# facebookresearch/EgoT2

Measured on NVIDIA B200. Metric: translator fwd+bwd clips/sec, higher is better.
Workload: dtype bf16

## Files before the change

### egot2_b200/_lib.py

```python
from __future__ import annotations

import ctypes as C
import os

MAX_SEG = 8
MAX_GROUPS = 4
F32, BF16 = 0, 1
LOSS_NONE, LOSS_CE, LOSS_BCE_SIGMOID, LOSS_CE_GROUPS = 0, 1, 2, 3
LR_CONSTANT, LR_COSINE, LR_STEPS = 0, 1, 2
LR_MAX_MILESTONES = 8

_LIB_PATH = os.environ.get("EGOT2_LIB") or os.path.join(os.path.dirname(os.path.abspath(__file__)), "lib", "libegot2.so")

i32, u64, f32, vp, sz = C.c_int32, C.c_uint64, C.c_float, C.c_void_p, C.c_size_t


class EmbedDesc(C.Structure):
    _fields_ = [("dtype", i32), ("feat_dtype", i32), ("B", i32), ("T", i32), ("H", i32), ("n_seg", i32),
                ("seg_tokens", i32 * MAX_SEG), ("seg_in_dim", i32 * MAX_SEG), ("seg_offset", i32 * MAX_SEG),
                ("seg_has_proj", i32 * MAX_SEG), ("training", i32), ("p_feat", f32), ("p_embed", f32),
                ("ln_eps", f32), ("seed", u64), ("no_ln", i32), ("feat_drop_tokens", i32)]


class EmbedIn(C.Structure):
    _fields_ = [("feat", vp * MAX_SEG), ("proj_w", vp * MAX_SEG), ("proj_b", vp * MAX_SEG), ("ln_g", vp),
                ("ln_b", vp), ("tok_table", vp)]


class EmbedOut(C.Structure):
    _fields_ = [("z", vp), ("stat", vp), ("x", vp)]


class EmbedGrads(C.Structure):
    _fields_ = [("proj_w", vp * MAX_SEG), ("proj_b", vp * MAX_SEG), ("ln_g", vp), ("ln_b", vp), ("tok_table", vp),
                ("dfeat", vp * MAX_SEG), ("seg_embed", vp * MAX_SEG)]


class LayerDesc(C.Structure):
    _fields_ = [("dtype", i32), ("B", i32), ("T", i32), ("H", i32), ("FF", i32), ("heads", i32), ("training", i32),
                ("layer_index", i32), ("p_drop", f32), ("ln_eps", f32), ("seed", u64)]


_LAYER_FIELDS = ["in_proj_w", "out_proj_w", "lin1_w", "lin2_w", "in_proj_b", "out_proj_b", "lin1_b", "lin2_b",
                 "norm1_g", "norm1_b", "norm2_g", "norm2_b"]


class LayerParams(C.Structure):
    _fields_ = [(n, vp) for n in _LAYER_FIELDS]


class LayerGrads(C.Structure):
    _fields_ = [(n, vp) for n in _LAYER_FIELDS]


class LayerSaved(C.Structure):
    _fields_ = [(n, vp) for n in ["qkv", "attn", "lse", "y1", "stat1", "x1", "hid", "y2", "stat2", "hid_mask", "ffn_scratch"]]


class DecoderDesc(C.Structure):
    _fields_ = [("dtype", i32), ("rows", i32), ("S", i32), ("mem_rows", i32), ("M", i32), ("kv_inner", i32),
                ("kv_outer", i32), ("kv_jstride", i32), ("kv_istride", i32), ("H", i32), ("FF", i32), ("heads", i32),
                ("training", i32), ("layer_index", i32), ("p_drop", f32), ("ln_eps", f32), ("seed", u64)]


_DEC_FIELDS = ["sa_in_w", "sa_out_w", "ca_in_w", "ca_out_w", "lin1_w", "lin2_w", "sa_in_b", "sa_out_b", "ca_in_b",
               "ca_out_b", "lin1_b", "lin2_b", "norm1_g", "norm1_b", "norm2_g", "norm2_b", "norm3_g", "norm3_b"]


class DecoderParams(C.Structure):
    _fields_ = [(n, vp) for n in _DEC_FIELDS]


class DecoderGrads(C.Structure):
    _fields_ = [(n, vp) for n in _DEC_FIELDS]


class DecoderSaved(C.Structure):
    _fields_ = [(n, vp) for n in ["qkv", "a1", "y1", "stat1", "x1", "qc", "kvc", "a2", "y2", "stat2", "x2", "hid", "y3",
                                  "stat3"]]


class HeadDesc(C.Structure):
    _fields_ = [("dtype", i32), ("B", i32), ("T", i32), ("H", i32), ("pool", i32), ("row_tokens", i32),
                ("use_ln", i32), ("n_out", i32), ("loss", i32), ("n_groups", i32), ("group_size", i32 * MAX_GROUPS),
                ("sub_rows", i32), ("training", i32), ("p_head", f32), ("ln_eps", f32), ("seed", u64)]


class HeadIn(C.Structure):
    _fields_ = [(n, vp) for n in ["x", "ln_g", "ln_b", "w", "b", "labels", "class_weight"]]


class HeadOut(C.Structure):
    _fields_ = [(n, vp) for n in ["pooled", "stat", "g", "logits", "loss", "argmax", "row_loss"]]


class DpDesc(C.Structure):
    _fields_ = [("world", i32), ("rank", i32), ("numel", C.c_int64), ("slab", vp * 8), ("off_param", C.c_int64),
                ("off_grad", C.c_int64), ("off_shadow", C.c_int64), ("off_flags", C.c_int64), ("exp_avg", vp), ("exp_avg_sq", vp),
                ("lr", f32), ("beta1", f32), ("beta2", f32), ("eps", f32), ("weight_decay", f32), ("step", i32), ("step_dev", vp),
                ("decoupled", i32), ("zero_grads_remote", i32), ("lr_dev", vp), ("guard", vp)]


class GradGuard(C.Structure):
    _fields_ = [("max_norm", f32), ("total_norm", f32), ("coef", f32), ("skip", i32), ("skipped", i32)]


class LrSched(C.Structure):
    _fields_ = [("kind", i32), ("n_milestones", i32), ("warmup_steps", C.c_int64), ("total_steps", C.c_int64),
                ("base_lr", C.c_double), ("warmup_start_lr", C.c_double), ("end_lr", C.c_double),
                ("milestones", C.c_int64 * LR_MAX_MILESTONES), ("factors", C.c_double * (LR_MAX_MILESTONES + 1))]


class HeadGrads(C.Structure):
    _fields_ = [(n, vp) for n in ["ln_g", "ln_b", "w", "b"]]


class VitDesc(C.Structure):
    _fields_ = [("dtype", i32), ("B", i32), ("T", i32), ("D", i32), ("heads", i32), ("dim_head", i32), ("mlp", i32),
                ("layer_index", i32), ("ln_eps", f32)]


_VIT_PARAM_FIELDS = ["qkv_w", "out_w", "ff1_w", "ff2_w", "norm_a_g", "norm_a_b", "norm_f_g", "norm_f_b", "ff1_b", "ff2_b"]


class VitParams(C.Structure):
    _fields_ = [(n, vp) for n in _VIT_PARAM_FIELDS]


class VitGrads(C.Structure):
    _fields_ = [(n, vp) for n in _VIT_PARAM_FIELDS]


class VitSaved(C.Structure):
    _fields_ = [(n, vp) for n in ["h", "stat_a", "qkv", "attn", "lse", "x1", "h2", "stat_f", "u", "act"]]


P = C.POINTER

SIGNATURES = {
    "egot2_version": (C.c_char_p, []),
    "egot2_last_error": (C.c_char_p, []),
    "egot2_sm_count": (C.c_int, []),
    "egot2_launch_count": (C.c_uint64, []),
    "egot2_dropout_epoch_enable": (C.c_int, [C.c_int]),
    "egot2_dropout_epoch_set": (C.c_int, [u64, vp]),
    "egot2_dropout_epoch_advance": (C.c_int, [vp]),
    "egot2_dropout_epoch_host": (C.c_int, [u64]),
    "egot2_pnr_metrics": (C.c_int, [i32, i32, vp, vp, vp, vp, vp, vp, vp, vp, vp, vp, vp, vp]),
    "egot2_row_softmax": (C.c_int, [C.c_int64, i32, vp, vp, vp]),
    "egot2_segment_softmax_mean": (C.c_int, [i32, i32, vp, vp, vp, vp]),
    "egot2_topk_correct": (C.c_int, [i32, i32, vp, vp, i32, vp, vp, vp]),
    "egot2_edit_distance_prefix": (C.c_int, [i32, i32, i32, vp, vp, vp, vp, vp]),
    "egot2_prof_enable": (C.c_int, [C.c_int]),
    "egot2_peer_alloc": (C.c_int, [C.c_size_t, C.POINTER(vp)]),
    "egot2_peer_free": (C.c_int, [vp]),
    "egot2_peer_handle_bytes": (C.c_int, []),
    "egot2_peer_export": (C.c_int, [vp, vp]),
    "egot2_peer_import": (C.c_int, [vp, C.POINTER(vp)]),
    "egot2_peer_unimport": (C.c_int, [vp]),
    "egot2_dp_flag_bytes": (C.c_size_t, []),
    "egot2_dp_reduce_adam": (C.c_int, [vp, vp]),
    "egot2_dp_reduce_adam_range": (C.c_int, [vp, C.c_int64, C.c_int64, i32, vp]),
    "egot2_side_defer": (C.c_int, [C.c_int]),
    "egot2_side_join_all": (C.c_int, [vp]),
    "egot2_timeline_set": (C.c_int, [vp]),
    "egot2_prof_report": (C.c_int, [C.c_char_p, sz]),
    "egot2_embed_workspace_bytes": (sz, [P(EmbedDesc), C.c_int]),
    "egot2_embed_fwd": (C.c_int, [P(EmbedDesc), P(EmbedIn), P(EmbedOut), vp, sz, vp]),
    "egot2_embed_bwd": (C.c_int, [P(EmbedDesc), P(EmbedIn), P(EmbedOut), vp, P(EmbedGrads), vp, sz, vp]),
    "egot2_hhi_tok_table_fwd": (C.c_int, [vp, vp, i32, i32, P(i32), P(i32), i32, vp, vp]),
    "egot2_hhi_tok_table_bwd": (C.c_int, [vp, i32, P(i32), P(i32), i32, vp, vp]),
    "egot2_ffn_scratch_bytes": (sz, [i32]),
    "egot2_encoder_layer_workspace_bytes": (sz, [P(LayerDesc), C.c_int]),
    "egot2_encoder_layer_fwd": (C.c_int, [P(LayerDesc), P(LayerParams), vp, vp, P(LayerSaved), vp, sz, vp]),
    "egot2_encoder_layer_bwd": (C.c_int, [P(LayerDesc), P(LayerParams), vp, P(LayerSaved), vp, vp, P(LayerGrads),
                                          vp, sz, vp]),
    "egot2_decoder_layer_workspace_bytes": (sz, [P(DecoderDesc)]),
    "egot2_decoder_layer_fwd": (C.c_int, [P(DecoderDesc), P(DecoderParams), vp, vp, vp, P(DecoderSaved), vp]),
    "egot2_decoder_layer_bwd": (C.c_int, [P(DecoderDesc), P(DecoderParams), vp, vp, P(DecoderSaved), vp, vp, vp,
                                          P(DecoderGrads), vp, sz, vp]),
    "egot2_vit_layer_workspace_bytes": (sz, [P(VitDesc)]),
    "egot2_vit_layer_fwd": (C.c_int, [P(VitDesc), P(VitParams), vp, vp, P(VitSaved), vp]),
    "egot2_vit_layer_bwd": (C.c_int, [P(VitDesc), P(VitParams), vp, P(VitSaved), vp, vp, P(VitGrads), vp, sz, vp]),
    "egot2_prompt_embed_fwd": (C.c_int, [i32, i32, i32, i32, vp, vp, vp, f32, i32, u64, vp, vp]),
    "egot2_prompt_embed_bwd": (C.c_int, [i32, i32, i32, i32, vp, vp, f32, i32, u64, vp, vp]),
    "egot2_head_rows": (C.c_int, [P(HeadDesc)]),
    "egot2_head_workspace_bytes": (sz, [P(HeadDesc)]),
    "egot2_head_loss_fwd": (C.c_int, [P(HeadDesc), P(HeadIn), P(HeadOut), vp]),
    "egot2_head_loss_bwd": (C.c_int, [P(HeadDesc), P(HeadIn), P(HeadOut), vp, f32, vp, P(HeadGrads), vp, sz, vp]),
    "egot2_slowfast_pool_fwd": (C.c_int, [vp, i32, i32, i32, i32, i32, i32, vp, i32, vp]),
    "egot2_cast_f32_to_bf16": (C.c_int, [vp, vp, sz, vp]),
    "egot2_sum_into_f32": (C.c_int, [vp, vp, vp, sz, vp]),
    "egot2_cast_bf16_to_f32": (C.c_int, [vp, vp, sz, vp]),
    "egot2_adam_step": (C.c_int, [vp, vp, vp, vp, sz, f32, f32, f32, f32, f32, i32, f32, vp]),
    "egot2_adam_step_fused": (C.c_int, [vp, vp, vp, vp, sz, f32, f32, f32, f32, f32, i32, f32, vp, i32, vp]),
    "egot2_adamw_step_fused": (C.c_int, [vp, vp, vp, vp, sz, f32, f32, f32, f32, f32, i32, f32, vp, i32, vp]),
    "egot2_adam_step_fused_dev": (C.c_int, [vp, vp, vp, vp, sz, f32, f32, f32, f32, f32, vp, f32, vp, i32, vp]),
    "egot2_adam_step_fused_sched": (C.c_int, [vp, vp, vp, vp, sz, vp, f32, f32, f32, f32, vp, f32, vp, i32, i32, vp]),
    "egot2_opt_advance": (C.c_int, [vp, vp, vp, vp]),
    "egot2_grad_norm_workspace_bytes": (sz, []),
    "egot2_grad_norm": (C.c_int, [vp, sz, f32, vp, vp, vp, sz, vp]),
    "egot2_adam_step_fused_guard": (C.c_int, [vp, vp, vp, vp, sz, f32, vp, f32, f32, f32, f32, vp, f32, vp, i32, i32, vp, vp]),
    "egot2_gemm": (C.c_int, [i32, i32, i32, i32, vp, i32, vp, i32, vp, i32, vp, i32, i32, vp]),
    "egot2_gemm_last_impl": (C.c_char_p, []),
    "egot2_layernorm_fwd": (C.c_int, [i32, i32, i32, vp, vp, vp, f32, vp, vp, vp]),
    "egot2_attention_fwd": (C.c_int, [i32, i32, i32, i32, i32, vp, vp, vp, f32, i32, u64, vp]),
    "egot2_attention_bwd": (C.c_int, [i32, i32, i32, i32, i32, vp, vp, vp, vp, vp, f32, i32, u64, vp, sz, vp]),
    "egot2_attention_bwd_workspace_bytes": (sz, [i32, i32, i32, i32, i32]),
    "egot2_pool_fwd": (C.c_int, [i32, i32, i32, i32, i32, i32, vp, vp, vp]),
    "egot2_pool_bwd": (C.c_int, [i32, i32, i32, i32, i32, i32, vp, vp, vp]),
}

_lib = None


class Egot2Error(RuntimeError):
    pass


def lib_path() -> str:
    return _LIB_PATH


def load():
    global _lib
    if _lib is not None:
        return _lib
    if not os.path.exists(_LIB_PATH):
        raise Egot2Error(f"{_LIB_PATH} not found: build it with `python -m egot2_b200.build` "
                         "(the CUDA library is mandatory; there is no PyTorch/CPU fallback)")
    lib = C.CDLL(_LIB_PATH)
    for name, (res, args) in SIGNATURES.items():
        fn = getattr(lib, name)
        fn.restype = res
        fn.argtypes = args
    _lib = lib
    return lib


def check(rc: int, what: str = ""):
    if rc != 0:
        msg = load().egot2_last_error().decode(errors="replace")
        raise Egot2Error(f"{what or 'egot2 call'} failed (rc={rc}): {msg}")


def call(name: str, *args):
    check(getattr(load(), name)(*args), name)


def prof_enable(on: bool = True):
    check(load().egot2_prof_enable(1 if on else 0), "egot2_prof_enable")


def prof_report():
    buf = C.create_string_buffer(1 << 20)
    check(load().egot2_prof_report(buf, len(buf)), "egot2_prof_report")
    rows = []
    for line in buf.value.decode().splitlines():
        tag, n, us = line.split("\t")
        rows.append((tag, int(n), float(us)))
    return sorted(rows, key=lambda r: -r[2])
```

### egot2_b200/csrc/api.cu

```cuda
#include <stdarg.h>
#include <stdlib.h>
#include <string.h>

#define EGOT2_FILE_ID 11
#include "ops.h"

namespace egot2 {

static thread_local char g_err[512] = "";
unsigned long long g_launch_count = 0;

void set_error(const char* fmt, ...) {
  va_list ap;
  va_start(ap, fmt);
  vsnprintf(g_err, sizeof(g_err), fmt, ap);
  va_end(ap);
}

#ifdef EGOT2_TIMELINE
static void (*g_tl_setters[32])(unsigned long long*);
static int g_tl_n = 0;
void tl_register(void (*setter)(unsigned long long*)) { if (g_tl_n < 32) g_tl_setters[g_tl_n++] = setter; }
#endif

unsigned long long g_host_epoch = 0;
static void (*g_epoch_setters[32])(const unsigned long long*);
static int g_epoch_n = 0;
void epoch_register(void (*setter)(const unsigned long long*)) { if (g_epoch_n < 32) g_epoch_setters[g_epoch_n++] = setter; }
namespace {
__global__ void epoch_advance_kernel(unsigned long long* slot, unsigned long long add) {
  EGOT2_PDL_ENTER();
  if (threadIdx.x == 0 && blockIdx.x == 0) *slot += add;
}
constexpr int kMaxDev = 64;
unsigned long long* g_epoch_slots[kMaxDev] = {};
int cur_dev() { int d = 0; return (cudaGetDevice(&d) == cudaSuccess && d >= 0 && d < kMaxDev) ? d : 0; }
#define g_epoch_slot (g_epoch_slots[cur_dev()])
}

bool pdl_enabled() {
  static const bool on = !(getenv("EGOT2_PDL") && atoi(getenv("EGOT2_PDL")) == 0);
  return on;
}

int sm_count() {
  static int cached[64] = {0};
  int dev = 0;
  if (cudaGetDevice(&dev) != cudaSuccess || dev < 0 || dev >= 64) return 148;
  if (cached[dev] == 0) {
    int n = 0;
    if (cudaDeviceGetAttribute(&n, cudaDevAttrMultiProcessorCount, dev) != cudaSuccess || n <= 0) n = 148;
    cached[dev] = n;
  }
  return cached[dev];
}

int suggest_split_k(int M, int N, int K) {
  const int tile = (M <= 64 || N <= 64) ? 64 : 128;
  const long long tiles = (long long)((M + tile - 1) / tile) * ((N + tile - 1) / tile);
  long long want = (2LL * sm_count() + tiles - 1) / tiles;
  long long max_by_k = K / 128;
  if (want > max_by_k) want = max_by_k;
  if (want < 1) want = 1;
  if (want > 64) want = 64;
  return (int)want;
}

namespace {
struct ProfRec { char tag[96]; cudaEvent_t e0, e1; };
constexpr int kProfMax = 16384;
ProfRec* g_prof = nullptr;
int g_prof_n = 0;
bool g_prof_on = false;
}
bool prof_enabled() { return g_prof_on; }
ProfScope::ProfScope(cudaStream_t stream, const char* fmt, ...) : st(stream), slot(-1) {
  static const bool trace = getenv("EGOT2_TRACE_LAUNCH") != nullptr;
  if (trace) {
    char tag[96];
    va_list ap;
    va_start(ap, fmt);
    vsnprintf(tag, sizeof(tag), fmt, ap);
    va_end(ap);
    fprintf(stderr, "[egot2] %s\n", tag);
    fflush(stderr);
  }
  if (!g_prof_on || g_prof_n >= kProfMax) return;
  cudaStreamCaptureStatus cs = cudaStreamCaptureStatusNone;
  if (cudaStreamIsCapturing(stream, &cs) != cudaSuccess || cs != cudaStreamCaptureStatusNone) return;
  ProfRec& r = g_prof[g_prof_n];
  if (!r.e0) { if (cudaEventCreate(&r.e0) != cudaSuccess || cudaEventCreate(&r.e1) != cudaSuccess) return; }
  va_list ap;
  va_start(ap, fmt);
  vsnprintf(r.tag, sizeof(r.tag), fmt, ap);
  va_end(ap);
  slot = g_prof_n++;
  cudaEventRecord(r.e0, st);
}
ProfScope::~ProfScope() {
  if (slot >= 0) cudaEventRecord(g_prof[slot].e1, st);
}

static thread_local const char* g_gemm_impl = "none";
const char* gemm_last_impl() { return g_gemm_impl; }

static int gemm_impl_mode() {
  static int mode = -1;
  if (mode < 0) {
    const char* e = getenv("EGOT2_GEMM");
    mode = (e && strcmp(e, "simt") == 0) ? 1 : 0;
  }
  return mode;
}

int gemm(const GemmArgs& a, cudaStream_t st) {
  if (a.in_dtype == EGOT2_BF16 && gemm_impl_mode() == 0) {
    const int rc = gemm_sm100(a, st);
    if (rc >= 0) { if (rc == 0) g_gemm_impl = "tcgen05"; return rc; }
  }
  g_gemm_impl = "simt";
  EGOT2_CHECK(!a.trans_c, "gemm: transposed accumulation exists in the tcgen05 kernel only");
  EGOT2_CHECK(a.ln_g == nullptr, "gemm: a fused LayerNorm was requested but the tcgen05 kernel did not take the problem");
  if (a.split_stride > 0) {
    GemmArgs b = a;
    b.split_k = 1; b.split_stride = 0;
    if (a.splits_out) *a.splits_out = 1;
    return gemm_simt(b, st);
  }
  return gemm_simt(a, st);
}

static bool env_is(const char* name, const char* value) {
  const char* e = getenv(name);
  return e && strcmp(e, value) == 0;
}

static bool force_simt_attention() {
  static int mode = -1;
  if (mode < 0) { const char* e = getenv("EGOT2_ATTN"); mode = (e && strcmp(e, "simt") == 0) ? 1 : 0; }
  return mode == 1;
}

int attention_fwd(int dtype, int B, int T, int H, int heads, const void* qkv, void* out, float* lse, float p_drop,
                  uint64_t drop_key, cudaStream_t st) {
  if (heads > 0 && H % heads == 0 && H / heads > 128)
    return attention_wide_fwd(dtype, B, T, H, heads, qkv, out, lse, p_drop, drop_key, st);
  if (attention_mma_supported(dtype, T, H, heads) && !force_simt_attention())
    return attention_mma_fwd(B, T, H, heads, qkv, out, lse, p_drop, drop_key, st);
  if (attention_long_supported(dtype, T, H, heads) && !force_simt_attention())
    return attention_long_fwd(B, T, H, heads, qkv, out, lse, p_drop, drop_key, st);
  return attention_simt_fwd(dtype, B, T, H, heads, qkv, out, lse, p_drop, drop_key, st);
}
int attention_bwd(int dtype, int B, int T, int H, int heads, const void* qkv, const void* out, const float* lse,
                  const void* dout, void* dqkv, float p_drop, uint64_t drop_key, void* ws, size_t ws_bytes,
                  cudaStream_t st) {
  if (heads > 0 && H % heads == 0 && H / heads > 128)
    return attention_wide_bwd(dtype, B, T, H, heads, qkv, out, lse, dout, dqkv, p_drop, drop_key, st);
  if (attention_mma_supported(dtype, T, H, heads) && !force_simt_attention())
    return attention_mma_bwd(B, T, H, heads, qkv, out, lse, dout, dqkv, p_drop, drop_key, st);
  if (attention_long_supported(dtype, T, H, heads) && !force_simt_attention())
    return attention_long_bwd(B, T, H, heads, qkv, out, lse, dout, dqkv, p_drop, drop_key, st);
  return attention_simt_bwd(dtype, B, T, H, heads, qkv, out, lse, dout, dqkv, p_drop, drop_key, ws, ws_bytes, st);
}

namespace {

struct Carver {
  char* base; size_t size, off = 0;
  Carver(void* p, size_t n) : base((char*)p), size(n) {}
  void* take(size_t bytes) {
    void* r = base ? base + off : nullptr;
    off += align_up(bytes);
    return r;
  }
  bool ok() const { return off <= size && (base != nullptr || off == 0); }
};

struct Side {
  cudaStream_t s = nullptr;
  cudaEvent_t fork[8] = {};
  cudaEvent_t join = nullptr;
  cudaEvent_t pend[2] = {};
  const void* pend_ws[2] = {nullptr, nullptr};
  int pend_next = 0;
  bool dirty = false;
};
int g_side_defer[kMaxDev] = {};
constexpr int kCallers = 4;
struct SideSets {
  Side sides[kCallers][3];
  cudaStream_t owner[kCallers] = {};
  unsigned long long used[kCallers] = {};
  unsigned long long tick = 0;
  int state = 0;
};
SideSets g_side_sets[kMaxDev];
Side* get_side(int idx, cudaStream_t caller) {
  SideSets& ss = g_side_sets[cur_dev()];
  if (ss.state == 0) {
    ss.state = 1;
    if (env_is("EGOT2_STREAMS", "0")) ss.state = -1;
    for (int c = 0; c < kCallers && ss.state == 1; ++c)
      for (int i = 0; i < 3 && ss.state == 1; ++i) {
        Side& sd = ss.sides[c][i];
        if (cudaStreamCreateWithFlags(&sd.s, cudaStreamNonBlocking) != cudaSuccess) ss.state = -1;
        for (int k = 0; k < 8 && ss.state == 1; ++k)
          if (cudaEventCreateWithFlags(&sd.fork[k], cudaEventDisableTiming) != cudaSuccess) ss.state = -1;
        if (ss.state == 1 && cudaEventCreateWithFlags(&sd.join, cudaEventDisableTiming) != cudaSuccess) ss.state = -1;
        for (int k = 0; k < 2 && ss.state == 1; ++k)
          if (cudaEventCreateWithFlags(&sd.pend[k], cudaEventDisableTiming) != cudaSuccess) ss.state = -1;
      }
  }
  if (ss.state != 1) return nullptr;
  int slot = -1, lru = 0;
  for (int c = 0; c < kCallers; ++c) {
    if (ss.used[c] && ss.owner[c] == caller) { slot = c; break; }
    if (ss.used[c] < ss.used[lru]) lru = c;
  }
  if (slot < 0) { slot = lru; ss.owner[slot] = caller; }
  ss.used[slot] = ++ss.tick;
  return &ss.sides[slot][idx];
}
}
int launch_priority(cudaStream_t st) {
  static int state = 0, lo = 0, hi = 0;
  if (state == 0) {
    state = 1;
    if (env_is("EGOT2_PRIO", "0") || cudaDeviceGetStreamPriorityRange(&lo, &hi) != cudaSuccess || lo == hi) state = -1;
  }
  if (state != 1) return INT_MIN;
  {
    const SideSets& ss = g_side_sets[cur_dev()];
    if (ss.state == 1)
      for (int c = 0; c < kCallers; ++c)
        for (int i = 0; i < 3; ++i)
          if (ss.sides[c][i].s == st) return lo;
  }
  return hi;
}
namespace {
cudaStream_t side_fork(cudaStream_t main, Side* sd, int k) {
  if (!sd || prof_enabled()) return main;
  if (cudaEventRecord(sd->fork[k], main) != cudaSuccess || cudaStreamWaitEvent(sd->s, sd->fork[k], 0) != cudaSuccess) return main;
  return sd->s;
}
int side_join(cudaStream_t main, Side* sd) {
  if (!sd || prof_enabled()) return 0;
  EGOT2_CUDA(cudaEventRecord(sd->join, sd->s));
  EGOT2_CUDA(cudaStreamWaitEvent(main, sd->join, 0));
  sd->dirty = false;
  sd->pend_ws[0] = sd->pend_ws[1] = nullptr;
  return 0;
}
bool side_deferred() { return g_side_defer[cur_dev()] != 0 && !prof_enabled(); }
int side_mark_pending(Side* sd, const void* ws) {
  if (!sd) return 0;
  int slot = sd->pend_ws[0] == ws ? 0 : sd->pend_ws[1] == ws ? 1 : (sd->pend_next++ & 1);
  EGOT2_CUDA(cudaEventRecord(sd->pend[slot], sd->s));
  sd->pend_ws[slot] = ws;
  sd->dirty = true;
  return 0;
}
int side_wait_pending(cudaStream_t main, Side* sd, const void* ws) {
  if (!sd) return 0;
  for (int k = 0; k < 2; ++k)
    if (sd->pend_ws[k] == ws) {
      EGOT2_CUDA(cudaStreamWaitEvent(main, sd->pend[k], 0));
      sd->pend_ws[k] = nullptr;
    }
  return 0;
}

int wgrad(int dtype, int rows, int n_out, int k_in, const void* dY, int ld_dy, int dy_rpg, int dy_gs, const void* X,
          int ld_x, int x_rpg, int x_gs, float* dW, cudaStream_t st, int share = 1) {
  static const bool swap_on = !env_is("EGOT2_WGRAD_SWAP", "0");
  if (swap_on && dtype == EGOT2_BF16 && gemm_impl_mode() == 0 && k_in <= 128 && n_out >= 512 && !dy_rpg && !x_rpg && share == 1) {
    GemmArgs t;
    t.M = k_in; t.N = n_out; t.K = rows;
    t.A = X; t.lda = ld_x; t.trans_a = 1;
    t.B = dY; t.ldb = ld_dy; t.trans_b = 0;
    t.C = dW; t.ldc = k_in; t.trans_c = 1; t.in_dtype = dtype; t.out_dtype = EGOT2_F32; t.accumulate = 1;
    t.split_k = suggest_split_k(t.M, t.N, t.K);
    const int rc = t.split_k >= 2 ? gemm_sm100(t, st) : -3;
    if (rc >= 0) return rc;
  }
  GemmArgs g;
  g.M = n_out; g.N = k_in; g.K = rows;
  g.A = dY; g.lda = ld_dy; g.trans_a = 1; g.a_rpg = dy_rpg; g.a_gstride = dy_gs;
  g.B = X; g.ldb = ld_x; g.trans_b = 0; g.b_rpg = x_rpg; g.b_gstride = x_gs;
  g.C = dW; g.ldc = k_in; g.in_dtype = dtype; g.out_dtype = EGOT2_F32; g.accumulate = 1;
  g.split_k = suggest_split_k(g.M, g.N, g.K);
  if (share > 1) g.split_k = g.split_k / share > 0 ? g.split_k / share : 1;
  return gemm(g, st);
}

}
}

using namespace egot2;

extern "C" const char* egot2_version(void) { return "egot2-b200 0.1 (sm_100a)"; }
extern "C" const char* egot2_last_error(void) { return g_err; }
extern "C" int egot2_sm_count(void) { return sm_count(); }
extern "C" uint64_t egot2_launch_count(void) { return g_launch_count; }

extern "C" int egot2_timeline_set(void* dev_buf) {
#ifdef EGOT2_TIMELINE
  for (int i = 0; i < g_tl_n; ++i) g_tl_setters[i]((unsigned long long*)dev_buf);
  return 0;
#else
  (void)dev_buf;
  EGOT2_CHECK(false, "this build has no timeline support (compile with -DEGOT2_TIMELINE)");
#endif
}

extern "C" int egot2_dropout_epoch_enable(int on) {
  if (on && !g_epoch_slot) {
    EGOT2_CUDA(cudaMalloc(&g_epoch_slot, sizeof(unsigned long long)));
    EGOT2_CUDA(cudaMemset(g_epoch_slot, 0, sizeof(unsigned long long)));
  }
  const unsigned long long* p = on ? g_epoch_slot : nullptr;
  for (int i = 0; i < g_epoch_n; ++i) g_epoch_setters[i](p);
  EGOT2_CUDA(cudaGetLastError());
  return 0;
}
extern "C" int egot2_dropout_epoch_set(uint64_t value, void* stream) {
  EGOT2_CHECK(g_epoch_slot != nullptr, "dropout epoch: call egot2_dropout_epoch_enable(1) first");
  EGOT2_CUDA(cudaMemsetAsync(g_epoch_slot, 0, sizeof(unsigned long long), (cudaStream_t)stream));
  if (value) {
    launch(epoch_advance_kernel, dim3(1), dim3(32), 0, (cudaStream_t)stream, g_epoch_slot, (unsigned long long)value);
    EGOT2_LAUNCH_CHECK();
  }
  return 0;
}
extern "C" int egot2_dropout_epoch_advance(void* stream) {
  EGOT2_CHECK(g_epoch_slot != nullptr, "dropout epoch: call egot2_dropout_epoch_enable(1) first");
  launch(epoch_advance_kernel, dim3(1), dim3(32), 0, (cudaStream_t)stream, g_epoch_slot, 1ull);
  EGOT2_LAUNCH_CHECK();
  return 0;
}
extern "C" int egot2_dropout_epoch_host(uint64_t value) { g_host_epoch = value; return 0; }

extern "C" int egot2_pnr_metrics(int32_t B, int32_t n, const float* logits, const int64_t* label_idx,
                                 const float* label_onehot, const int64_t* sc_label, const double* fps,
                                 const int64_t* start_frame, const int64_t* end_frame, const int64_t* pnr_frame,
                                 double* err_sec, int64_t* out_counts, double* out_dist_sum, void* stream) {
  return pnr_metrics(B, n, logits, label_idx, label_onehot, sc_label, fps, start_frame, end_frame, pnr_frame, err_sec,
                     (long long*)out_counts, out_dist_sum, (cudaStream_t)stream);
}

extern "C" int egot2_prof_enable(int on) {
  if (on && !g_prof) {
    g_prof = (ProfRec*)calloc(kProfMax, sizeof(ProfRec));
    EGOT2_CHECK(g_prof != nullptr, "prof: out of host memory");
  }
  g_prof_on = on != 0;
  if (on) g_prof_n = 0;
  return 0;
}
extern "C" int egot2_prof_report(char* buf, size_t buf_bytes) {
  EGOT2_CHECK(buf && buf_bytes > 0, "prof_report: no buffer");
  struct Agg { const char* tag; int n; double us; };
  Agg* agg = (Agg*)calloc(g_prof_n > 0 ? g_prof_n : 1, sizeof(Agg));
  int na = 0;
  for (int i = 0; i < g_prof_n; ++i) {
    float ms = 0.f;
    EGOT2_CUDA(cudaEventSynchronize(g_prof[i].e1));
    EGOT2_CUDA(cudaEventElapsedTime(&ms, g_prof[i].e0, g_prof[i].e1));
    int j = 0;
    for (; j < na; ++j) if (strcmp(agg[j].tag, g_prof[i].tag) == 0) break;
    if (j == na) { agg[na].tag = g_prof[i].tag; agg[na].n = 0; agg[na].us = 0; ++na; }
    agg[j].n += 1; agg[j].us += ms * 1e3;
  }
  size_t off = 0;
  buf[0] = 0;
  for (int j = 0; j < na; ++j) {
    int w = snprintf(buf + off, buf_bytes - off, "%s\t%d\t%.3f\n", agg[j].tag, agg[j].n, agg[j].us);
    if (w < 0 || (size_t)w >= buf_bytes - off) break;
    off += w;
  }
  free(agg);
  return 0;
}

namespace {
void seg_stream_plan(const egot2_embed_desc* d, int* idx) {
  long long load[3] = {0, 0, 0};
  bool done[EGOT2_MAX_SEG] = {};
  for (int it = 0; it < d->n_seg; ++it) {
    int best = -1;
    long long bc = -1;
    for (int k = 0; k < d->n_seg; ++k) {
      if (done[k]) continue;
      const long long c = d->seg_has_proj[k] ? (long long)d->seg_in_dim[k] * d->seg_tokens[k] : 1;
      if (c > bc) { bc = c; best = k; }
    }
    int sidx = 0;
    for (int j = 1; j < 3; ++j) if (load[j] < load[sidx]) sidx = j;
    idx[best] = sidx;
    load[sidx] += bc;
    done[best] = true;
  }
}

bool embed_splitk(const egot2_embed_desc* d) {
  if (env_is("EGOT2_EMBED_SPLITK", "0")) return false;
  if (d->no_ln || !embed_finish_supported(d->dtype, d->H)) return false;
  if (env_is("EGOT2_EMBED_SPLITK", "1")) return true;
  for (int k = 0; k < d->n_seg; ++k) {
    if (!d->seg_has_proj[k] || d->seg_tokens[k] == 0) continue;
    const long long tiles = (((long long)d->B * d->seg_tokens[k] + 127) / 128) * ((d->H + 127) / 128);
    if (d->seg_in_dim[k] >= 2048 && tiles * 2 <= sm_count()) return true;
  }
  return false;
}
int embed_seg_splits(const egot2_embed_desc* d, int k) {
  if (!d->seg_has_proj[k] || d->seg_tokens[k] == 0) return 1;
  const long long tiles = (((long long)d->B * d->seg_tokens[k] + 127) / 128) * ((d->H + 127) / 128);
  long long s = sm_count() / tiles;
  if (s > d->seg_in_dim[k] / 512) s = d->seg_in_dim[k] / 512;
  if (s > 16) s = 16;
  return s < 1 ? 1 : (int)s;
}
size_t embed_slab_floats(const egot2_embed_desc* d) {
  size_t n = 0;
  for (int k = 0; k < d->n_seg; ++k)
    if (d->seg_has_proj[k]) n += (size_t)embed_seg_splits(d, k) * d->B * d->seg_tokens[k] * d->H;
  return n;
}
}

extern "C" size_t egot2_embed_workspace_bytes(const egot2_embed_desc* d, int backward) {
  size_t n = 256;
  if (!backward && embed_splitk(d)) n += align_up(embed_slab_floats(d) * 4);
  if (!backward && d->feat_dtype != d->dtype) {
    size_t mx = 0;
    for (int k = 0; k < d->n_seg; ++k) {
      const size_t e = (size_t)d->B * d->seg_tokens[k] * d->seg_in_dim[k];
      if (e > mx) mx = e;
    }
    n += align_up(mx * dtype_size(d->dtype));
  }
  if (backward && d->feat_dtype != d->dtype) {
    size_t mx = 0;
    for (int k = 0; k < d->n_seg; ++k) {
      const size_t e = (size_t)d->B * d->seg_tokens[k] * d->seg_in_dim[k];
      if (e > mx) mx = e;
    }
    n += align_up(mx * dtype_size(d->dtype));
  }
  if (backward) n += align_up((size_t)d->B * d->T * d->H * dtype_size(d->dtype));
  return n;
}

static int embed_check(const egot2_embed_desc* d) {
  EGOT2_CHECK(d->n_seg >= 1 && d->n_seg <= EGOT2_MAX_SEG, "embed: n_seg=%d out of range", d->n_seg);
  EGOT2_CHECK(d->dtype == EGOT2_F32 || d->dtype == EGOT2_BF16, "embed: bad dtype %d", d->dtype);
  EGOT2_CHECK(d->feat_dtype == d->dtype || (d->feat_dtype == EGOT2_F32 && d->dtype == EGOT2_BF16),
              "embed: features must be in the compute dtype, or fp32 with bf16 compute");
  int tot = 0;
  for (int k = 0; k < d->n_seg; ++k) {
    EGOT2_CHECK(d->seg_offset[k] == tot, "embed: segment %d offset %d != running total %d", k, d->seg_offset[k], tot);
    EGOT2_CHECK(d->seg_has_proj[k] || d->seg_in_dim[k] == d->H, "embed: pass-through segment %d must be H wide", k);
    tot += d->seg_tokens[k];
  }
  EGOT2_CHECK(tot == d->T, "embed: segments cover %d tokens, T=%d", tot, d->T);
  EGOT2_CHECK(!d->no_ln || !d->training || (d->p_feat == 0.f && d->p_embed == 0.f),
              "embed: the LayerNorm-free variant has no dropout sites (p_feat=%f p_embed=%f)", d->p_feat, d->p_embed);
  return 0;
}

extern "C" int egot2_embed_fwd(const egot2_embed_desc* d, const egot2_embed_in* in, const egot2_embed_out* out,
                               void* workspace, size_t ws_bytes, void* stream) {
  cudaStream_t st = (cudaStream_t)stream;
  EGOT2_TRY(embed_check(d));
  if (d->B == 0 || d->T == 0) return 0;
  const size_t es = dtype_size(d->dtype);
  Carver ws(workspace, ws_bytes);
  void* cast_buf = nullptr;
  const bool splitk = embed_splitk(d);
  float* zf = nullptr;
  EmbedSrc src;
  src.n = d->n_seg;
  if (splitk) {
    zf = (float*)ws.take(embed_slab_floats(d) * 4);
    EGOT2_CHECK(ws.ok(), "embed_fwd: workspace too small (%zu < %zu)", ws_bytes, ws.off);
  }
  if (d->feat_dtype != d->dtype) {
    size_t mx = 0;
    for (int k = 0; k < d->n_seg; ++k) {
      const size_t e = (size_t)d->B * d->seg_tokens[k] * d->seg_in_dim[k];
      if (e > mx) mx = e;
    }
    cast_buf = ws.take(mx * dtype_size(d->dtype));
    EGOT2_CHECK(ws.ok(), "embed_fwd: workspace too small (%zu < %zu)", ws_bytes, ws.off);
  }
  const bool par = d->feat_dtype == d->dtype;
  Side* sides[2] = {par ? get_side(0, st) : nullptr, par ? get_side(1, st) : nullptr};
  bool used[2] = {false, false};
  cudaStream_t side_st[2] = {st, st};
  int seg_idx[EGOT2_MAX_SEG] = {};
  seg_stream_plan(d, seg_idx);
  for (int i = 0; i < 2 && i + 1 < d->n_seg; ++i)
    if (sides[i]) { side_st[i] = side_fork(st, sides[i], 0); used[i] = side_st[i] != st; }
  bool ln_fused = !splitk && !d->no_ln && d->dtype == EGOT2_BF16 && d->feat_dtype == EGOT2_BF16 && d->H == 128 &&
                  !(d->training && d->p_feat > 0.f) && gemm_impl_mode() == 0 && env_is("EGOT2_GEMM_LN", "1");
  for (int k = 0; k < d->n_seg && ln_fused; ++k)
    if (d->seg_tokens[k] > 0 && (!d->seg_has_proj[k] || d->seg_in_dim[k] % 8 != 0)) ln_fused = false;
  for (int k = 0; k < d->n_seg; ++k) {
    const int Dk = d->seg_tokens[k], Kk = d->seg_in_dim[k];
    if (Dk == 0) continue;
    cudaStream_t sk = seg_idx[k] > 0 ? side_st[seg_idx[k] - 1] : st;
    char* zk = (char*)out->z + (size_t)d->seg_offset[k] * d->H * es;
    const void* feat = in->feat[k];
    if (splitk && !d->seg_has_proj[k]) {
      src.direct[k] = feat; src.direct_f32[k] = d->feat_dtype == EGOT2_F32 && d->dtype != EGOT2_F32;
      continue;
    }
    if (d->feat_dtype != d->dtype) {
      EGOT2_TRY(cast_f32_to(d->dtype, (const float*)feat, cast_buf, (size_t)d->B * Dk * Kk, sk));
      feat = cast_buf;
    }
    if (d->seg_has_proj[k]) {
      GemmArgs g;
      g.M = d->B * Dk; g.N = d->H; g.K = Kk;
      g.A = feat; g.lda = Kk;
      g.B = in->proj_w[k]; g.ldb = Kk; g.trans_b = 1;
      g.C = zk; g.ldc = d->H; g.c_rpg = Dk; g.c_gstride = d->T;
      g.bias = in->proj_b[k];
      g.in_dtype = d->dtype; g.out_dtype = d->dtype;
      if (splitk) {
        g.C = zf; g.ldc = d->H; g.c_rpg = 0; g.c_gstride = 0; g.out_dtype = EGOT2_F32;
        g.split_k = embed_seg_splits(d, k); g.split_stride = (long long)d->B * Dk * d->H;
        int used = 1;
        g.splits_out = &used;
        EGOT2_TRY(gemm(g, sk));
        src.slab[k] = zf; src.splits[k] = used;
        zf += (size_t)embed_seg_splits(d, k) * d->B * Dk * d->H;
      } else {
        if (ln_fused) {
          g.ln_g = in->ln_g; g.ln_b = in->ln_b; g.ln_eps = d->ln_eps;
          g.ln_out = (char*)out->x + (size_t)d->seg_offset[k] * d->H * es; g.ln_stat = out->stat;
          g.ln_table = in->tok_table; g.ln_table_rows = d->T; g.ln_row0 = d->seg_offset[k];
          if (d->training && d->p_embed > 0.f) { g.ln_p_drop = d->p_embed; g.ln_drop_key = site_key(d->seed, SITE_EMBED, 0); }
          if (!gemm_sm100_ln_ok(g)) {
            ln_fused = false;
            g.ln_g = nullptr; g.ln_b = nullptr; g.ln_out = nullptr; g.ln_stat = nullptr; g.ln_table = nullptr; g.ln_p_drop = 0.f;
          }
        }
        EGOT2_TRY(gemm(g, sk));
      }
    } else {
      EGOT2_CUDA(cudaMemcpy2DAsync(zk, (size_t)d->T * d->H * es, feat, (size_t)Dk * d->H * es, (size_t)Dk * d->H * es,
                                   d->B, cudaMemcpyDeviceToDevice, sk));
    }
  }
  for (int i = 0; i < 2; ++i) if (used[i]) EGOT2_TRY(side_join(st, sides[i]));
  const size_t n = (size_t)d->B * d->T * d->H;
  if (splitk) {
    for (int k = 0; k < d->n_seg; ++k) { src.tok_begin[k] = d->seg_offset[k]; src.tokens[k] = d->seg_tokens[k]; }
    return embed_finish(d->B, d->T, d->H, src, (d->feat_drop_tokens > 0 && d->feat_drop_tokens < d->T) ? d->feat_drop_tokens : 0,
                        d->training ? d->p_feat : 0.f, site_key(d->seed, SITE_FEAT, 0), in->ln_g, in->ln_b, d->ln_eps, in->tok_table,
                        d->training ? d->p_embed : 0.f, site_key(d->seed, SITE_EMBED, 0), out->z, out->stat, out->x, st);
  }
  if (d->training && d->p_feat > 0.f) {
    if (d->feat_drop_tokens > 0 && d->feat_drop_tokens < d->T)
      EGOT2_TRY(dropout_prefix_inplace(d->dtype, out->z, n, (size_t)d->T * d->H, (size_t)d->feat_drop_tokens * d->H, d->p_feat,
                                       site_key(d->seed, SITE_FEAT, 0), st));
    else
      EGOT2_TRY(dropout_inplace(d->dtype, out->z, n, d->p_feat, site_key(d->seed, SITE_FEAT, 0), st));
  }
  if (d->no_ln) return add_table(d->dtype, n, (size_t)d->T * d->H, out->z, in->tok_table, out->x, st);
  if (ln_fused) return 0;
  LayerNormArgs l;
  l.rows = d->B * d->T; l.H = d->H; l.dtype = d->dtype; l.x = out->z; l.g = in->ln_g; l.b = in->ln_b; l.eps = d->ln_eps;
  l.y = out->x; l.stat = out->stat; l.table = in->tok_table; l.table_rows = d->T;
  if (d->training && d->p_embed > 0.f) { l.p_drop = d->p_embed; l.drop_key = site_key(d->seed, SITE_EMBED, 0); }
  return layernorm_fwd(l, st);
}

extern "C" int egot2_embed_bwd(const egot2_embed_desc* d, const egot2_embed_in* in, const egot2_embed_out* saved,
                               const void* dx_c, const egot2_embed_grads* g, void* workspace, size_t ws_bytes,
                               void* stream) {
  cudaStream_t st = (cudaStream_t)stream;
  EGOT2_TRY(embed_check(d));
  if (d->B == 0 || d->T == 0) return 0;
  void* dx = const_cast<void*>(dx_c);
  const size_t es = dtype_size(d->dtype);
  const size_t n = (size_t)d->B * d->T * d->H;
  Carver ws(workspace, ws_bytes);
  void* cast_buf = nullptr;
  if (d->feat_dtype != d->dtype) {
    size_t mx = 0;
    for (int k = 0; k < d->n_seg; ++k) {
      const size_t e = (size_t)d->B * d->seg_tokens[k] * d->seg_in_dim[k];
      if (e > mx) mx = e;
    }
    cast_buf = ws.take(mx * es);
  }
  void* dz = ws.take(n * es);
  EGOT2_CHECK(ws.ok(), "embed_bwd: workspace too small (%zu < %zu)", ws_bytes, ws.off);
  const float pe = (d->training && d->p_embed > 0.f) ? d->p_embed : 0.f;
  const uint64_t ke = site_key(d->seed, SITE_EMBED, 0);
  SegOut so;
  so.n = d->n_seg;
  bool want_table = g->tok_table != nullptr;
  for (int k = 0; k < d->n_seg; ++k) { so.tokens[k] = d->seg_tokens[k]; so.out[k] = g->seg_embed[k]; want_table |= g->seg_embed[k] != nullptr; }
  Side* tside = want_table ? get_side(2, st) : nullptr;
  if (want_table) EGOT2_TRY(table_grad(d->dtype, d->B, d->T, d->H, dx, g->tok_table, so, pe, ke, side_fork(st, tside, 0)));
  if (d->no_ln) {
    dz = dx;
  } else {
    LayerNormBwdArgs l;
    l.rows = d->B * d->T; l.H = d->H; l.dtype = d->dtype; l.x = saved->z; l.stat = saved->stat; l.g = in->ln_g;
    l.dy = dx; l.dx = dz; l.dg = g->ln_g; l.db = g->ln_b; l.dy_p_drop = pe; l.dy_drop_key = ke;
    EGOT2_TRY(layernorm_bwd(l, st));
    if (d->training && d->p_feat > 0.f) {
      if (d->feat_drop_tokens > 0 && d->feat_drop_tokens < d->T)
        EGOT2_TRY(dropout_prefix_inplace(d->dtype, dz, n, (size_t)d->T * d->H, (size_t)d->feat_drop_tokens * d->H, d->p_feat,
                                         site_key(d->seed, SITE_FEAT, 0), st));
      else
        EGOT2_TRY(dropout_inplace(d->dtype, dz, n, d->p_feat, site_key(d->seed, SITE_FEAT, 0), st));
    }
  }
  const bool par = d->feat_dtype == d->dtype;
  Side* sides[2] = {par ? get_side(0, st) : nullptr, par ? get_side(1, st) : nullptr};
  bool used[2] = {false, false};
  cudaStream_t side_st[2] = {st, st};
  int seg_idx[EGOT2_MAX_SEG] = {};
  seg_stream_plan(d, seg_idx);
  for (int i = 0; i < 2 && i + 1 < d->n_seg; ++i)
    if (sides[i]) { side_st[i] = side_fork(st, sides[i], 0); used[i] = side_st[i] != st; }
  int n_proj = 0, n_big = 0;
  long long sum_big = 0;
  for (int k = 0; k < d->n_seg; ++k) {
    const bool on = d->seg_has_proj[k] && d->seg_tokens[k] > 0;
    n_proj += on ? 1 : 0;
    n_big += (on && d->seg_in_dim[k] >= 2048) ? 1 : 0;
    if (on && d->seg_in_dim[k] >= 2048) sum_big += (long long)d->seg_in_dim[k] * d->seg_tokens[k];
  }
  const int share_all = n_big > 0 ? n_big : n_proj;
  auto big_share = [&](int Kk, int Dk) {
    const long long w = (long long)Kk * Dk;
    const long long sh = w > 0 ? (sum_big + w / 2) / w : 1;
    return (int)(sh < 1 ? 1 : sh);
  };
  bool bias_on_main = false;
  SegOut sb_main;
  {
    SegOut sb;
    sb.n = d->n_seg;
    bool any = false;
    for (int k = 0; k < d->n_seg; ++k) {
      sb.tokens[k] = d->seg_tokens[k];
      sb.out[k] = (d->seg_has_proj[k] && d->seg_tokens[k] > 0) ? g->proj_b[k] : nullptr;
      any |= sb.out[k] != nullptr;
    }
    Side* bside = get_side(2, st);
    if (any && tside) {
      bias_on_main = true;
      sb_main = sb;
    } else if (any) {
      EGOT2_TRY(table_grad(d->dtype, d->B, d->T, d->H, dz, nullptr, sb, 0.f, 0, side_fork(st, bside, 1)));
      if (bside && !tside) tside = bside;
    }
  }
  for (int k = 0; k < d->n_seg; ++k) {
    const int Dk = d->seg_tokens[k], Kk = d->seg_in_dim[k];
    if (Dk == 0) continue;
    cudaStream_t sk = seg_idx[k] > 0 ? side_st[seg_idx[k] - 1] : st;
    const char* dzk = (const char*)dz + (size_t)d->seg_offset[k] * d->H * es;
    if (d->seg_has_proj[k]) {
      const void* feat = in->feat[k];
      if (d->feat_dtype != d->dtype) {
        EGOT2_TRY(cast_f32_to(d->dtype, (const float*)feat, cast_buf, (size_t)d->B * Dk * Kk, sk));
        feat = cast_buf;
      }
      if (g->proj_w[k])
        EGOT2_TRY(wgrad(d->dtype, d->B * Dk, d->H, Kk, dzk, d->H, Dk, d->T, feat, Kk, 0, 0, g->proj_w[k], sk,
                        !par ? 1 : ((n_big > 0 && Kk < 2048) ? 8 : (n_big > 0 ? big_share(Kk, Dk) : share_all))));
      if (g->dfeat[k]) {
        GemmArgs m;
        m.M = d->B * Dk; m.N = Kk; m.K = d->H;
        m.A = dzk; m.lda = d->H; m.a_rpg = Dk; m.a_gstride = d->T;
        m.B = in->proj_w[k]; m.ldb = Kk; m.trans_b = 0;
        m.C = g->dfeat[k]; m.ldc = Kk; m.in_dtype = d->dtype; m.out_dtype = EGOT2_F32;
        EGOT2_TRY(gemm(m, sk));
      }
    } else if (g->dfeat[k]) {
      if (d->dtype == EGOT2_F32) {
        EGOT2_CUDA(cudaMemcpy2DAsync(g->dfeat[k], (size_t)Dk * d->H * 4, dzk, (size_t)d->T * d->H * 4,
                                     (size_t)Dk * d->H * 4, d->B, cudaMemcpyDeviceToDevice, sk));
      } else {
        for (int b = 0; b < d->B; ++b)
          EGOT2_TRY(cast_to_f32(d->dtype, dzk + (size_t)b * d->T * d->H * es, g->dfeat[k] + (size_t)b * Dk * d->H,
                                (size_t)Dk * d->H, sk));
      }
    }
  }
  if (bias_on_main) EGOT2_TRY(table_grad(d->dtype, d->B, d->T, d->H, dz, nullptr, sb_main, 0.f, 0, st));
  for (int i = 0; i < 2; ++i) if (used[i]) EGOT2_TRY(side_join(st, sides[i]));
  if (tside) EGOT2_TRY(side_join(st, tside));
  return 0;
}

namespace {
struct LayerWs {
  void *d1, *d2, *d3, *d4, *d5, *dhid, *dqkv, *attn_ws;
  size_t attn_ws_bytes;
};
size_t layer_ws_layout(const egot2_layer_desc* d, int backward, void* base, size_t bytes, LayerWs* out) {
  Carver ws(base, bytes);
  if (backward) {
    const size_t es = dtype_size(d->dtype);
    const size_t M = (size_t)d->B * d->T;
    LayerWs w;
    w.d1 = ws.take(M * d->H * es);
    w.d2 = ws.take(M * d->H * es);
    w.d3 = ws.take(M * d->H * es);
    w.d4 = ws.take(M * d->H * es);
    w.d5 = ws.take(M * d->H * es);
    w.dhid = ws.take(M * d->FF * es);
    w.dqkv = ws.take(M * 3 * d->H * es);
    w.attn_ws_bytes = attention_bwd_workspace(d->dtype, d->B, d->T, d->H, d->heads);
    w.attn_ws = ws.take(w.attn_ws_bytes);
    if (out) *out = w;
  }
  return ws.off + 256;
}
int layer_check(const egot2_layer_desc* d) {
  EGOT2_CHECK(d->dtype == EGOT2_F32 || d->dtype == EGOT2_BF16, "layer: bad dtype %d", d->dtype);
  EGOT2_CHECK(d->heads > 0 && d->H % d->heads == 0, "layer: H=%d not divisible by heads=%d", d->H, d->heads);
  EGOT2_CHECK(d->p_drop >= 0.f && d->p_drop < 1.f, "layer: dropout p=%f out of [0,1)", d->p_drop);
  return 0;
}
}

extern "C" size_t egot2_ffn_scratch_bytes(int32_t M) { return M > 0 ? ffn_scratch_bytes(M) : 0; }

extern "C" size_t egot2_encoder_layer_workspace_bytes(const egot2_layer_desc* d, int backward) {
  return layer_ws_layout(d, backward, nullptr, 0, nullptr);
}

extern "C" int egot2_encoder_layer_fwd(const egot2_layer_desc* d, const egot2_layer_params* p, const void* x_in,
                                       void* x_out, const egot2_layer_saved* s, void* workspace, size_t ws_bytes,
                                       void* stream) {
  (void)workspace; (void)ws_bytes;
  cudaStream_t st = (cudaStream_t)stream;
  EGOT2_TRY(layer_check(d));
  const int M = d->B * d->T, H = d->H, FF = d->FF;
  if (M == 0) return 0;
  const float pd = d->training ? d->p_drop : 0.f;
  const uint32_t L = (uint32_t)d->layer_index;
  bool ln1_fused = false;
  {
    GemmArgs g; g.M = M; g.N = 3 * H; g.K = H; g.A = x_in; g.lda = H; g.B = p->in_proj_w; g.ldb = H; g.trans_b = 1;
    g.C = s->qkv; g.ldc = 3 * H; g.bias = p->in_proj_b; g.in_dtype = d->dtype; g.out_dtype = d->dtype;
    EGOT2_TRY(gemm(g, st));
  }
  EGOT2_TRY(attention_fwd(d->dtype, d->B, d->T, H, d->heads, s->qkv, s->attn, s->lse, pd, site_key(d->seed, SITE_ATTN, L), st));
  {
    GemmArgs g; g.M = M; g.N = H; g.K = H; g.A = s->attn; g.lda = H; g.B = p->out_proj_w; g.ldb = H; g.trans_b = 1;
    g.C = s->y1; g.ldc = H; g.bias = p->out_proj_b; g.residual = x_in; g.ldr = H;
    g.p_drop = pd; g.drop_key = site_key(d->seed, SITE_DROP1, L); g.in_dtype = d->dtype; g.out_dtype = d->dtype;
    g.ln_g = p->norm1_g; g.ln_b = p->norm1_b; g.ln_eps = d->ln_eps; g.ln_out = s->x1; g.ln_stat = s->stat1;
    ln1_fused = d->dtype == EGOT2_BF16 && gemm_sm100_ln_ok(g) && !env_is("EGOT2_GEMM", "simt");
    if (!ln1_fused) { g.ln_g = nullptr; g.ln_b = nullptr; g.ln_out = nullptr; g.ln_stat = nullptr; }
    EGOT2_TRY(gemm(g, st));
  }
  if (!ln1_fused) {
    LayerNormArgs l; l.rows = M; l.H = H; l.dtype = d->dtype; l.x = s->y1; l.g = p->norm1_g; l.b = p->norm1_b;
    l.eps = d->ln_eps; l.y = s->x1; l.stat = s->stat1;
    EGOT2_TRY(layernorm_fwd(l, st));
  }
  if (ffn_fused_supported(d->dtype, H, FF) && !env_is("EGOT2_FFN", "unfused"))
    return ffn_fused_fwd(M, FF, s->x1, p->lin1_w, p->lin1_b, p->lin2_w, p->lin2_b, p->norm2_g, p->norm2_b, d->ln_eps,
                         s->hid, s->hid_mask, s->y2, s->stat2, x_out, pd, site_key(d->seed, SITE_FFN, L),
                         site_key(d->seed, SITE_DROP2, L), s->ffn_scratch, st);
  {
    GemmArgs g; g.M = M; g.N = FF; g.K = H; g.A = s->x1; g.lda = H; g.B = p->lin1_w; g.ldb = H; g.trans_b = 1;
    g.C = s->hid; g.ldc = FF; g.bias = p->lin1_b; g.relu = 1;
    g.p_drop = pd; g.drop_key = site_key(d->seed, SITE_FFN, L); g.drop_bit_mode = 1; g.in_dtype = d->dtype; g.out_dtype = d->dtype;
    EGOT2_TRY(gemm(g, st));
  }
  {
    GemmArgs g; g.M = M; g.N = H; g.K = FF; g.A = s->hid; g.lda = FF; g.B = p->lin2_w; g.ldb = FF; g.trans_b = 1;
    g.C = s->y2; g.ldc = H; g.bias = p->lin2_b; g.residual = s->x1; g.ldr = H;
    g.p_drop = pd; g.drop_key = site_key(d->seed, SITE_DROP2, L); g.in_dtype = d->dtype; g.out_dtype = d->dtype;
    EGOT2_TRY(gemm(g, st));
  }
  {
    LayerNormArgs l; l.rows = M; l.H = H; l.dtype = d->dtype; l.x = s->y2; l.g = p->norm2_g; l.b = p->norm2_b;
    l.eps = d->ln_eps; l.y = x_out; l.stat = s->stat2;
    EGOT2_TRY(layernorm_fwd(l, st));
  }
  return 0;
}

extern "C" int egot2_encoder_layer_bwd(const egot2_layer_desc* d, const egot2_layer_params* p, const void* x_in,
                                       const egot2_layer_saved* s, void* dx_out, void* dx_in,
                                       const egot2_layer_grads* g, void* workspace, size_t ws_bytes, void* stream) {
  cudaStream_t st = (cudaStream_t)stream;
  EGOT2_TRY(layer_check(d));
  const int M = d->B * d->T, H = d->H, FF = d->FF;
  if (M == 0) return 0;
  LayerWs w;
  const size_t need = layer_ws_layout(d, 1, workspace, ws_bytes, &w);
  EGOT2_CHECK(workspace && ws_bytes + 256 >= need, "encoder_layer_bwd: workspace too small (%zu < %zu)", ws_bytes, need);
  const size_t es = dtype_size(d->dtype);
  const float pd = d->training ? d->p_drop : 0.f;
  const float inv_keep = pd > 0.f ? 1.f / (1.f - pd) : 1.f;
  const uint32_t L = (uint32_t)d->layer_index;
  const int dt = d->dtype;

  Side* sd0 = get_side(0, st);
  Side* sd1 = get_side(1, st);
  Side* sd2 = get_side(2, st);
  const bool defer = side_deferred();
  if (defer) {
    EGOT2_TRY(side_wait_pending(st, sd0, workspace));
    EGOT2_TRY(side_wait_pending(st, sd1, workspace));
    EGOT2_TRY(side_wait_pending(st, sd2, workspace));
  }

  const void* d2 = w.d1;
  {
    LayerNormBwdArgs l; l.rows = M; l.H = H; l.dtype = dt; l.x = s->y2; l.stat = s->stat2; l.g = p->norm2_g;
    l.dy = dx_out; l.dx = w.d1; l.dg = g->norm2_g; l.db = g->norm2_b;
    if (pd > 0.f) { l.dx2 = w.d2; l.dx2_p_drop = pd; l.dx2_drop_key = site_key(d->seed, SITE_DROP2, L); d2 = w.d2; }
    l.dcol = g->lin2_b;
    EGOT2_TRY(layernorm_bwd(l, st));
  }
  static const bool late_wgrad = env_is("EGOT2_LATE_WGRAD", "1");
  auto fork_dw2 = [&]() -> int {
    cudaStream_t ss = side_fork(st, sd0, 0);
    return wgrad(dt, M, H, FF, d2, H, 0, 0, s->hid, FF, 0, 0, g->lin2_w, ss);
  };
  if (!late_wgrad) EGOT2_TRY(fork_dw2());
  const bool fused_dx = s->hid_mask && ffn_fused_supported(dt, H, FF) && !env_is("EGOT2_FFN", "unfused");
  if (fused_dx) {
    EGOT2_TRY(ffn_fused_bwd_dx(M, FF, d2, pd > 0.f ? w.d1 : nullptr, s->hid_mask, p->lin1_w, p->lin2_w, pd, w.dhid, w.d3, s->ffn_scratch,
                               g->lin1_b, st));
  } else {
    GemmArgs m; m.M = M; m.N = FF; m.K = H; m.A = d2; m.lda = H; m.B = p->lin2_w; m.ldb = FF; m.trans_b = 0;
    m.C = w.dhid; m.ldc = FF; m.mask = s->hid; m.ldm = FF; m.mask_scale = inv_keep; m.in_dtype = dt; m.out_dtype = dt;
    EGOT2_TRY(gemm(m, st));
    GemmArgs n; n.M = M; n.N = H; n.K = FF; n.A = w.dhid; n.lda = FF; n.B = p->lin1_w; n.ldb = H; n.trans_b = 0;
    n.C = w.d3; n.ldc = H; n.residual = w.d1; n.ldr = H; n.in_dtype = dt; n.out_dtype = dt;
    EGOT2_TRY(gemm(n, st));
  }
  auto fork_dw1 = [&]() -> int {
    cudaStream_t ss = side_fork(st, sd1, 1);
    EGOT2_TRY(wgrad(dt, M, FF, H, w.dhid, FF, 0, 0, s->x1, H, 0, 0, g->lin1_w, ss));
    if (!fused_dx) {
      cudaStream_t s2 = side_fork(st, sd2, 1);
      EGOT2_TRY(colsum_accum(dt, M, FF, w.dhid, FF, 0, 0, g->lin1_b, s2));
    }
    return 0;
  };
  if (!late_wgrad) EGOT2_TRY(fork_dw1());
  const void* dyo = w.d4;
  {
    LayerNormBwdArgs l; l.rows = M; l.H = H; l.dtype = dt; l.x = s->y1; l.stat = s->stat1; l.g = p->norm1_g;
    l.dy = w.d3; l.dx = w.d4; l.dg = g->norm1_g; l.db = g->norm1_b;
    if (pd > 0.f) { l.dx2 = w.d5; l.dx2_p_drop = pd; l.dx2_drop_key = site_key(d->seed, SITE_DROP1, L); dyo = w.d5; }
    l.dcol = g->out_proj_b;
    EGOT2_TRY(layernorm_bwd(l, st));
  }
  if (late_wgrad) { EGOT2_TRY(fork_dw2()); EGOT2_TRY(fork_dw1()); }
  {
    cudaStream_t ss = side_fork(st, sd2, 2);
    EGOT2_TRY(wgrad(dt, M, H, H, dyo, H, 0, 0, s->attn, H, 0, 0, g->out_proj_w, ss));
  }
  {
    GemmArgs m; m.M = M; m.N = H; m.K = H; m.A = dyo; m.lda = H; m.B = p->out_proj_w; m.ldb = H; m.trans_b = 0;
    m.C = w.d3; m.ldc = H; m.in_dtype = dt; m.out_dtype = dt;
    EGOT2_TRY(gemm(m, st));
  }
  EGOT2_TRY(attention_bwd(dt, d->B, d->T, H, d->heads, s->qkv, s->attn, s->lse, w.d3, w.dqkv, pd,
                          site_key(d->seed, SITE_ATTN, L), w.attn_ws, w.attn_ws_bytes, st));
  {
    cudaStream_t ss = side_fork(st, sd0, 3);
    EGOT2_TRY(wgrad(dt, M, 3 * H, H, w.dqkv, 3 * H, 0, 0, x_in, H, 0, 0, g->in_proj_w, ss));
    cudaStream_t s2 = side_fork(st, sd2, 3);
    EGOT2_TRY(colsum_accum(dt, M, 3 * H, w.dqkv, 3 * H, 0, 0, g->in_proj_b, s2));
  }
  {
    GemmArgs m; m.M = M; m.N = H; m.K = 3 * H; m.A = w.dqkv; m.lda = 3 * H; m.B = p->in_proj_w; m.ldb = H; m.trans_b = 0;
    m.C = dx_in; m.ldc = H; m.residual = w.d4; m.ldr = H; m.in_dtype = dt; m.out_dtype = dt;
    EGOT2_TRY(gemm(m, st));
  }
  if (defer) {
    EGOT2_TRY(side_mark_pending(sd0, workspace));
    EGOT2_TRY(side_mark_pending(sd1, workspace));
    return side_mark_pending(sd2, workspace);
  }
  EGOT2_TRY(side_join(st, sd0));
  EGOT2_TRY(side_join(st, sd1));
  return side_join(st, sd2);
}

extern "C" int egot2_side_defer(int on) { g_side_defer[cur_dev()] = on ? 1 : 0; return 0; }

extern "C" int egot2_side_join_all(void* stream) {
  SideSets& ss = g_side_sets[cur_dev()];
  if (ss.state == 1)
    for (int c = 0; c < kCallers; ++c)
      for (int i = 0; i < 3; ++i)
        if (ss.sides[c][i].dirty) EGOT2_TRY(side_join((cudaStream_t)stream, &ss.sides[c][i]));
  return 0;
}

extern "C" int egot2_head_rows(const egot2_head_desc* d) { return d->pool ? d->B : d->B * d->row_tokens; }

extern "C" size_t egot2_head_workspace_bytes(const egot2_head_desc* d) {
  const size_t rows = (size_t)egot2_head_rows(d), es = dtype_size(d->dtype);
  const size_t ldl = ((size_t)d->n_out + 7) / 8 * 8;
  return align_up(rows * ldl * es) + align_up(rows * d->H * es) + align_up(rows * d->H * 4) + 256;
}

extern "C" int egot2_head_loss_fwd(const egot2_head_desc* d, const egot2_head_in* in, const egot2_head_out* out,
                                   void* stream) {
  cudaStream_t st = (cudaStream_t)stream;
  const int rows = egot2_head_rows(d);
  if (rows == 0) return 0;
  EGOT2_CHECK(d->pool || (d->row_tokens > 0 && d->row_tokens <= d->T), "head: row_tokens=%d out of range", d->row_tokens);
  if (head_fused_supported(*d)) {
    if (d->loss != EGOT2_LOSS_NONE)
      EGOT2_CHECK(in->labels && out->row_loss && out->loss, "head_loss_fwd: labels/row_loss/loss buffers required");
    EGOT2_TRY(head_fused_fwd(*d, *in, *out, st));
    return loss_reduce(*d, rows, out->row_loss, out->loss, st);
  }
  EGOT2_TRY(pool_fwd(d->dtype, d->B, d->T, d->H, d->pool, d->row_tokens, in->x, out->pooled, st));
  const float ph = d->training ? d->p_head : 0.f;
  if (d->use_ln) {
    LayerNormArgs l; l.rows = rows; l.H = d->H; l.dtype = d->dtype; l.x = out->pooled; l.x_is_f32 = 1; l.g = in->ln_g;
    l.b = in->ln_b; l.eps = d->ln_eps; l.y = out->g; l.stat = out->stat;
    l.p_drop = ph; l.drop_key = site_key(d->seed, SITE_HEAD, 0);
    EGOT2_TRY(layernorm_fwd(l, st));
  } else {
    EGOT2_TRY(cast_f32_to(d->dtype, out->pooled, out->g, (size_t)rows * d->H, st));
    EGOT2_TRY(dropout_inplace(d->dtype, out->g, (size_t)rows * d->H, ph, site_key(d->seed, SITE_HEAD, 0), st));
  }
  {
    GemmArgs g; g.M = rows; g.N = d->n_out; g.K = d->H; g.A = out->g; g.lda = d->H; g.B = in->w; g.ldb = d->H; g.trans_b = 1;
    g.C = out->logits; g.ldc = d->n_out; g.bias = in->b; g.in_dtype = d->dtype; g.out_dtype = EGOT2_F32;
    EGOT2_TRY(gemm(g, st));
  }
  return loss_fwd(*d, rows, out->logits, in->labels, in->class_weight, out->row_loss, out->loss, out->argmax, st);
}

extern "C" int egot2_head_loss_bwd(const egot2_head_desc* d, const egot2_head_in* in, const egot2_head_out* saved,
                                   float* dlogits, float dloss_scale, void* dx, const egot2_head_grads* g,
                                   void* workspace, size_t ws_bytes, void* stream) {
  cudaStream_t st = (cudaStream_t)stream;
  const int rows = egot2_head_rows(d);
  if (rows == 0) return 0;
  const size_t es = dtype_size(d->dtype);
  if (head_fused_supported(*d))
    return head_fused_bwd(*d, *in, *saved, dlogits, dloss_scale, dx, *g, st);
  EGOT2_CHECK(workspace && ws_bytes >= egot2_head_workspace_bytes(d) - 256, "head_loss_bwd: workspace too small");
  Carver ws(workspace, ws_bytes);
  const int ldl = d->dtype == EGOT2_F32 ? d->n_out : (d->n_out + 7) / 8 * 8;
  void* dl_lp = ws.take((size_t)rows * ldl * es);
  void* dg = ws.take((size_t)rows * d->H * es);
  float* dpooled = (float*)ws.take((size_t)rows * d->H * 4);
  if (d->loss != EGOT2_LOSS_NONE)
    EGOT2_TRY(loss_bwd(*d, rows, saved->logits, in->labels, in->class_weight, saved->loss, dloss_scale, dlogits, st));
  const void* dl = dlogits;
  if (d->dtype != EGOT2_F32) {
    EGOT2_TRY(cast_rows_f32_to_bf16(dlogits, rows, d->n_out, dl_lp, ldl, st));
    dl = dl_lp;
  }
  if (g->w) EGOT2_TRY(wgrad(d->dtype, rows, d->n_out, d->H, dl, ldl, 0, 0, saved->g, d->H, 0, 0, g->w, st));
  if (g->b) EGOT2_TRY(colsum_accum(EGOT2_F32, rows, d->n_out, dlogits, d->n_out, 0, 0, g->b, st));
  const float ph = d->training ? d->p_head : 0.f;
  if (d->dtype == EGOT2_BF16 && !d->use_ln && d->n_out >= 2048 && !env_is("EGOT2_HEAD_SPLITK", "0")) {
    EGOT2_CUDA(cudaMemsetAsync(dpooled, 0, (size_t)rows * d->H * 4, st));
    GemmArgs m; m.M = rows; m.N = d->H; m.K = d->n_out; m.A = dl; m.lda = ldl; m.B = in->w; m.ldb = d->H; m.trans_b = 0;
    m.C = dpooled; m.ldc = d->H; m.in_dtype = d->dtype; m.out_dtype = EGOT2_F32; m.accumulate = 1;
    m.split_k = suggest_split_k(m.M, m.N, m.K);
    EGOT2_TRY(gemm(m, st));
    EGOT2_TRY(dropout_inplace(EGOT2_F32, dpooled, (size_t)rows * d->H, ph, site_key(d->seed, SITE_HEAD, 0), st));
    return pool_bwd(d->dtype, d->B, d->T, d->H, d->pool, d->row_tokens, dpooled, dx, st);
  }
  {
    GemmArgs m; m.M = rows; m.N = d->H; m.K = d->n_out; m.A = dl; m.lda = ldl; m.B = in->w; m.ldb = d->H; m.trans_b = 0;
    m.C = dg; m.ldc = d->H; m.in_dtype = d->dtype; m.out_dtype = d->dtype;
    EGOT2_TRY(gemm(m, st));
  }
  EGOT2_TRY(dropout_inplace(d->dtype, dg, (size_t)rows * d->H, ph, site_key(d->seed, SITE_HEAD, 0), st));
  if (d->use_ln) {
    LayerNormBwdArgs l; l.rows = rows; l.H = d->H; l.dtype = d->dtype; l.x = saved->pooled; l.x_is_f32 = 1;
    l.stat = saved->stat; l.g = in->ln_g; l.dy = dg; l.dy_is_f32 = (d->dtype == EGOT2_F32); l.dx = dpooled; l.dx_is_f32 = 1;
    l.dg = g->ln_g; l.db = g->ln_b;
    EGOT2_TRY(layernorm_bwd(l, st));
  } else {
    EGOT2_TRY(cast_to_f32(d->dtype, dg, dpooled, (size_t)rows * d->H, st));
  }
  return pool_bwd(d->dtype, d->B, d->T, d->H, d->pool, d->row_tokens, dpooled, dx, st);
}

extern "C" int egot2_gemm(int32_t dtype, int32_t M, int32_t N, int32_t K, const void* A, int32_t trans_a, const void* B,
                          int32_t trans_b, const float* bias, int32_t relu, void* C, int32_t c_is_f32,
                          int32_t accumulate, void* stream) {
  GemmArgs g;
  g.M = M; g.N = N; g.K = K;
  g.A = A; g.trans_a = trans_a; g.lda = trans_a ? M : K;
  g.B = B; g.trans_b = trans_b; g.ldb = trans_b ? K : N;
  g.C = C; g.ldc = N; g.bias = bias; g.relu = relu;
  g.in_dtype = dtype; g.out_dtype = c_is_f32 ? EGOT2_F32 : dtype; g.accumulate = accumulate;
  if (accumulate && !relu) g.split_k = suggest_split_k(M, N, K);
  return gemm(g, (cudaStream_t)stream);
}

extern "C" int egot2_sum_into_f32(float* dst, float* a, float* b, size_t n, void* stream) {
  return sum_into_clear(dst, a, b, n, (cudaStream_t)stream);
}

extern "C" const char* egot2_gemm_last_impl(void) { return gemm_last_impl(); }

extern "C" int egot2_attention_fwd(int32_t dtype, int32_t B, int32_t T, int32_t H, int32_t heads, const void* qkv,
                                   void* out, float* lse, float p_drop, int32_t training, uint64_t seed, void* stream) {
  return attention_fwd(dtype, B, T, H, heads, qkv, out, lse, training ? p_drop : 0.f, site_key(seed, SITE_ATTN, 0),
                       (cudaStream_t)stream);
}
extern "C" int egot2_attention_bwd(int32_t dtype, int32_t B, int32_t T, int32_t H, int32_t heads, const void* qkv,
                                   const void* out, const float* lse, const void* dout, void* dqkv, float p_drop,
                                   int32_t training, uint64_t seed, void* workspace, size_t ws_bytes, void* stream) {
  return attention_bwd(dtype, B, T, H, heads, qkv, out, lse, dout, dqkv, training ? p_drop : 0.f,
                       site_key(seed, SITE_ATTN, 0), workspace, ws_bytes, (cudaStream_t)stream);
}
extern "C" size_t egot2_attention_bwd_workspace_bytes(int32_t dtype, int32_t B, int32_t T, int32_t H, int32_t heads) {
  return attention_bwd_workspace(dtype, B, T, H, heads);
}
extern "C" int egot2_pool_fwd(int32_t dtype, int32_t B, int32_t T, int32_t H, int32_t pool, int32_t row_tokens,
                              const void* x, float* pooled, void* stream) {
  return pool_fwd(dtype, B, T, H, pool, row_tokens, x, pooled, (cudaStream_t)stream);
}
extern "C" int egot2_pool_bwd(int32_t dtype, int32_t B, int32_t T, int32_t H, int32_t pool, int32_t row_tokens,
                              const float* dpooled, void* dx, void* stream) {
  return pool_bwd(dtype, B, T, H, pool, row_tokens, dpooled, dx, (cudaStream_t)stream);
}
```

### egot2_b200/csrc/gemm_sm100.cu

```cuda
#include <stdio.h>
#include <stdlib.h>

#define EGOT2_FILE_ID 4
#include "ops.h"
#include "sm100.cuh"

namespace egot2 {

using namespace sm100;

namespace {

constexpr int BM = 128;
constexpr int BK = 64;
#ifndef EGOT2_GEMM_EPG
#define EGOT2_GEMM_EPG 1
#endif
constexpr int EPG = EGOT2_GEMM_EPG;
constexpr int NTHREADS = 64 + 128 * EPG;

struct EpiArgs {
  int M, N;
  void* C; int ldc; int c_rpg, c_gstride;
  const float* bias; int relu;
  const void* mask; int ldm; float mask_scale;
  float p_drop; uint64_t drop_key; int drop_bit_mode;
  const void* residual; int ldr;
  int accumulate; int atomic;
  long long split_stride;
  int tma_store;
  int k_grouped, kg, kdblocks;
  const float* ln_g; const float* ln_b; float ln_eps;
  void* ln_out; float* ln_stat; const float* ln_table; int ln_table_rows; int ln_row0;
  float ln_p_drop; uint64_t ln_drop_key;
  int trans_c;
  int tma_red;
  int trace_slot;
};

#ifdef EGOT2_GEMM_TRACE
__device__ long long g_gtrace[512][16];
#define GTR(k) do { if (blockIdx.x == 0 && blockIdx.z == 0 && e.trace_slot >= 0) g_gtrace[e.trace_slot][k] = clock64(); } while (0)
#else
#define GTR(k) do { } while (0)
#endif

__device__ __forceinline__ long long remap(int r, int rpg, int gstride) {
  return rpg > 0 ? (long long)(r / rpg) * gstride + (r % rpg) : (long long)r;
}


__device__ __forceinline__ void red_add_v4(float* p, float a, float b, float c, float d) {
  asm volatile("red.global.add.v4.f32 [%0], {%1, %2, %3, %4};" ::"l"(p), "f"(a), "f"(b), "f"(c), "f"(d) : "memory");
}

__device__ __forceinline__ bool aligned16(const void* p) { return (reinterpret_cast<uintptr_t>(p) & 15) == 0; }

__device__ __forceinline__ void load32(const float* p, float (&o)[32]) {
#pragma unroll
  for (int j = 0; j < 32; j += 4) {
    const float4 t = *reinterpret_cast<const float4*>(p + j);
    o[j] = t.x; o[j + 1] = t.y; o[j + 2] = t.z; o[j + 3] = t.w;
  }
}
__device__ __forceinline__ void load32(const bf16* p, float (&o)[32]) {
#pragma unroll
  for (int j = 0; j < 32; j += 8) {
    const uint4 t = *reinterpret_cast<const uint4*>(p + j);
    const uint32_t w[4] = {t.x, t.y, t.z, t.w};
#pragma unroll
    for (int k = 0; k < 4; ++k) {
      o[j + 2 * k] = __uint_as_float(w[k] << 16);
      o[j + 2 * k + 1] = __uint_as_float(w[k] & 0xffff0000u);
    }
  }
}
__device__ __forceinline__ void store32(float* p, const float (&v)[32]) {
#pragma unroll
  for (int j = 0; j < 32; j += 4) *reinterpret_cast<float4*>(p + j) = make_float4(v[j], v[j + 1], v[j + 2], v[j + 3]);
}
__device__ __forceinline__ void store32(bf16* p, const float (&v)[32]) {
#pragma unroll
  for (int j = 0; j < 32; j += 8) {
    uint4 o;
    __nv_bfloat162 p0 = __floats2bfloat162_rn(v[j], v[j + 1]), p1 = __floats2bfloat162_rn(v[j + 2], v[j + 3]);
    __nv_bfloat162 p2 = __floats2bfloat162_rn(v[j + 4], v[j + 5]), p3 = __floats2bfloat162_rn(v[j + 6], v[j + 7]);
    o.x = *reinterpret_cast<uint32_t*>(&p0); o.y = *reinterpret_cast<uint32_t*>(&p1);
    o.z = *reinterpret_cast<uint32_t*>(&p2); o.w = *reinterpret_cast<uint32_t*>(&p3);
    *reinterpret_cast<uint4*>(p + j) = o;
  }
}

template <int BN, typename TO> struct TileCfg {
  static constexpr uint32_t OUT_BYTES = (BN <= 128 && sizeof(TO) == 2) ? 128 * BN * 2 : 0;
  static constexpr int STAGES = BN == 128 ? (OUT_BYTES ? 2 : 3) : (BN == 64 ? (OUT_BYTES ? 3 : 4) : 4);
  static constexpr int MIN_CTAS = BN == 256 ? 1 : 2;
};
__device__ __forceinline__ void sts128(uint32_t dst, uint32_t a, uint32_t b, uint32_t c, uint32_t d) {
  asm volatile("st.shared.v4.b32 [%0], {%1, %2, %3, %4};" ::"r"(dst), "r"(a), "r"(b), "r"(c), "r"(d) : "memory");
}

__device__ __forceinline__ void named_bar_sync(int id, int n) { asm volatile("bar.sync %0, %1;" ::"r"(id), "r"(n) : "memory"); }

template <int BN, bool A_MN, bool B_MN, typename TO>
__global__ void __launch_bounds__(NTHREADS, TileCfg<BN, TO>::MIN_CTAS)
gemm_sm100_kernel(const __grid_constant__ CUtensorMap tma_a, const __grid_constant__ CUtensorMap tma_b,
                  const __grid_constant__ CUtensorMap tma_c, const EpiArgs e, const int k_blocks_total, const int k_blocks_per_split, const int tiles_n, const int num_tiles) {
  constexpr uint32_t A_BYTES = BM * BK * 2;
  constexpr uint32_t B_BYTES = BN * BK * 2;
  constexpr int STAGES = TileCfg<BN, TO>::STAGES;
  extern __shared__ uint8_t smem_raw[];
  const uint32_t smem_base = (smem_u32(smem_raw) + 1023u) & ~1023u;
  const uint32_t sA = smem_base;
  const uint32_t sB = sA + STAGES * A_BYTES;
  const uint32_t sOut = sB + STAGES * B_BYTES;
  const uint32_t bars = sOut + TileCfg<BN, TO>::OUT_BYTES;
  const uint32_t full0 = bars, empty0 = bars + 8 * STAGES, tmem_full = bars + 16 * STAGES, tmem_empty = tmem_full + 16;
  const uint32_t tmem_slot = tmem_empty + 16;
  const uint32_t bias_off = (tmem_slot + 8 + 15u) & ~15u;
  uint32_t* tmem_slot_ptr = reinterpret_cast<uint32_t*>(smem_raw + (tmem_slot - smem_u32(smem_raw)));

  const int warp = threadIdx.x >> 5, lane = threadIdx.x & 31;
  const int kb_begin = blockIdx.z * k_blocks_per_split;
  const int kb_end = min(k_blocks_total, kb_begin + k_blocks_per_split);
  const int nkb = kb_end - kb_begin;

  pdl_launch_dependents();
  if (threadIdx.x == 0) GTR(0);
  if (warp == 0 && lane == 0) {
    tma_prefetch_desc(&tma_a);
    tma_prefetch_desc(&tma_b);
    if (e.tma_store || e.tma_red) tma_prefetch_desc(&tma_c);
    for (int s = 0; s < STAGES; ++s) { mbar_init(full0 + 8 * s, 1); mbar_init(empty0 + 8 * s, 1); }
    for (int s = 0; s < 2; ++s) { mbar_init(tmem_full + 8 * s, 1); mbar_init(tmem_empty + 8 * s, 4 * EPG); }
    fence_barrier_init();
  }
  const bool one_tile = gridDim.z > 1;
  if (warp == 1) { if (one_tile) tmem_alloc<BN>(tmem_slot); else tmem_alloc<2 * BN>(tmem_slot); }
  if (threadIdx.x == 0) GTR(1);
  pdl_wait();
  if (threadIdx.x == 0) GTR(2);
  EGOT2_TL(EGOT2_FILE_ID);
  const unsigned long long egot2_ep = epoch_xor();
  float* sbias = reinterpret_cast<float*>(smem_raw + (bias_off - smem_u32(smem_raw)));
  tc_fence_before();
  __syncthreads();
  tc_fence_after();
  const uint32_t tmem_base = *tmem_slot_ptr;
  if (threadIdx.x == 0) GTR(3);

  if (warp == 0) {
    if (lane == 0) {
      int it = 0;
      for (int tile = blockIdx.x; tile < num_tiles; tile += gridDim.x) {
        const int m0 = (tile / tiles_n) * BM, n0 = (tile % tiles_n) * BN;
        for (int i = 0; i < nkb; ++i, ++it) {
          const int s = it % STAGES;
          const uint32_t ph = (it / STAGES) & 1;
          mbar_wait(empty0 + 8 * s, ph ^ 1);
          mbar_expect_tx(full0 + 8 * s, A_BYTES + B_BYTES);
          const int kb = kb_begin + i;
          const int k = kb * BK;
          if (A_MN && B_MN && e.k_grouped) {
            const int grp = (kb / e.kdblocks) * e.kg, d0 = (kb % e.kdblocks) * 64;
#pragma unroll
            for (int j = 0; j < BM / 64; ++j) tma_load_3d(sA + s * A_BYTES + j * 8192, &tma_a, full0 + 8 * s, m0 + 64 * j, d0, grp);
#pragma unroll
            for (int j = 0; j < BN / 64; ++j) tma_load_3d(sB + s * B_BYTES + j * 8192, &tma_b, full0 + 8 * s, n0 + 64 * j, d0, grp);
            continue;
          }
          if (!A_MN) {
            tma_load_2d(sA + s * A_BYTES, &tma_a, full0 + 8 * s, k, m0);
          } else {
#pragma unroll
            for (int j = 0; j < BM / 64; ++j) tma_load_2d(sA + s * A_BYTES + j * 8192, &tma_a, full0 + 8 * s, m0 + 64 * j, k);
          }
          if (!B_MN) {
            tma_load_2d(sB + s * B_BYTES, &tma_b, full0 + 8 * s, k, n0);
          } else {
#pragma unroll
            for (int j = 0; j < BN / 64; ++j) tma_load_2d(sB + s * B_BYTES + j * 8192, &tma_b, full0 + 8 * s, n0 + 64 * j, k);
          }
          if (tile == (int)blockIdx.x && (i == 0 || i == nkb - 1)) GTR(i == 0 ? 4 : 5);
        }
      }
    }
  } else if (warp == 1) {
    if (lane == 0) {
      constexpr uint32_t idesc = make_idesc_bf16(BM, BN, A_MN, B_MN);
      int it = 0, lt = 0;
      for (int tile = blockIdx.x; tile < num_tiles; tile += gridDim.x, ++lt) {
        const int buf = lt & 1;
        mbar_wait(tmem_empty + 8 * buf, ((lt >> 1) & 1) ^ 1);
        tc_fence_after();
        for (int i = 0; i < nkb; ++i, ++it) {
          const int s = it % STAGES;
          const uint32_t ph = (it / STAGES) & 1;
          mbar_wait(full0 + 8 * s, ph);
          if (lt == 0 && (i == 0 || i == nkb - 1)) GTR(i == 0 ? 6 : 7);
          tc_fence_after();
#pragma unroll
          for (int kk = 0; kk < BK / 16; ++kk) {
            const uint64_t ad = A_MN ? make_smem_desc_sw128(sA + s * A_BYTES + kk * 2048, 8192, 1024)
                                     : make_smem_desc_sw128(sA + s * A_BYTES + kk * 32, 16, 1024);
            const uint64_t bd = B_MN ? make_smem_desc_sw128(sB + s * B_BYTES + kk * 2048, 8192, 1024)
                                     : make_smem_desc_sw128(sB + s * B_BYTES + kk * 32, 16, 1024);
            umma_bf16(tmem_base + buf * BN, ad, bd, idesc, (i > 0 || kk > 0) ? 1u : 0u);
          }
          umma_commit(empty0 + 8 * s);
        }
        umma_commit(tmem_full + 8 * buf);
      }
    }
  } else {
    const int q = warp & 3;
    const int c_lo = ((warp - 2) >> 2) * (BN / EPG), c_hi = c_lo + BN / EPG;
    const float inv_keep = e.p_drop > 0.f ? 1.f / (1.f - e.p_drop) : 1.f;
    const bool first_split = blockIdx.z == 0;
    const float* bias = first_split ? e.bias : nullptr;
    const bool tma_red = sizeof(TO) == 4 && e.tma_red && gridDim.z > 1 && nkb > 0;
    int lt = 0;
    for (int tile = blockIdx.x; tile < num_tiles; tile += gridDim.x, ++lt) {
      const int buf = lt & 1;
      const int m0 = (tile / tiles_n) * BM, n0 = (tile % tiles_n) * BN;
      const int m = m0 + q * 32 + lane;
      float* sb = sbias + buf * BN;
      if (bias) {
        for (int i = threadIdx.x - 64; i < BN; i += NTHREADS - 64) sb[i] = n0 + i < e.N ? __ldg(bias + n0 + i) : 0.f;
        named_bar_sync(1, NTHREADS - 64);
      }
      const bool row_ok = (m < e.M) && nkb > 0;
      const long long crow = row_ok ? remap(m, e.c_rpg, e.c_gstride) : 0;
      TO* __restrict__ crow_ptr = (TO*)e.C + (long long)blockIdx.z * e.split_stride + crow * e.ldc;
      const TO* mask_row = e.mask ? (const TO*)e.mask + (long long)(row_ok ? m : 0) * e.ldm : nullptr;
      const TO* res_row = (e.residual && first_split) ? (const TO*)e.residual + (long long)(row_ok ? m : 0) * e.ldr : nullptr;
      const bool vec_ok = aligned16(crow_ptr) && aligned16(mask_row) && aligned16(res_row);
      const TO* aux_row = mask_row ? mask_row : res_row;
      float aux[32], aux_next[32];
      const bool aux_vec = row_ok && vec_ok && aux_row != nullptr;
      if (aux_vec && n0 + c_lo + 32 <= e.N) load32(aux_row + n0 + c_lo, aux_next);
      if (e.tma_store && lt > 0) {
        if (warp == 2 && lane == 0) tma_store_wait_read();
        named_bar_sync(3, NTHREADS - 64);
      }
      mbar_wait(tmem_full + 8 * buf, (lt >> 1) & 1);
      if (lt == 0 && threadIdx.x == 64) GTR(8);
      tc_fence_after();
      float ln_sum = 0.f, ln_sq = 0.f;
      if (tma_red) {
        const int rr = q * 32 + lane;
        uint32_t ra[32], rb[32];
        auto stage = [&](const uint32_t (&r)[32], int c0) {
          const uint32_t wbox = sA + (uint32_t)(c0 >> 5) * 16384u + (uint32_t)(q * 32) * 128u;
          if (e.trans_c) {
#pragma unroll
            for (int j = 0; j < 32; ++j)
              asm volatile("st.shared.b32 [%0], %1;" ::"r"(wbox + (uint32_t)j * 128u + (uint32_t)((((lane >> 2) ^ (j & 7)) << 4) | ((lane & 3) << 2))), "r"(r[j]) : "memory");
          } else {
            const uint32_t srow = wbox + (uint32_t)lane * 128u;
#pragma unroll
            for (int j = 0; j < 8; ++j) sts128(srow + (uint32_t)((j ^ (rr & 7)) << 4), r[4 * j], r[4 * j + 1], r[4 * j + 2], r[4 * j + 3]);
          }
          fence_proxy_async();
          __syncwarp();
          if (lane == 0 && n0 + c0 < e.N) {
            if (e.trans_c) tma_reduce_add_2d(&tma_c, wbox, m0 + q * 32, n0 + c0);
            else tma_reduce_add_2d(&tma_c, wbox, n0 + c0, m0 + q * 32);
          }
        };
        const uint32_t tcol = tmem_base + ((uint32_t)(q * 32) << 16) + (uint32_t)(buf * BN);
        tmem_ld_32x32(tcol + c_lo, ra);
#pragma unroll 1
        for (int c0 = c_lo; c0 < c_hi; c0 += 64) {
          tmem_ld_wait();
          if (c0 + 32 < c_hi) tmem_ld_32x32(tcol + c0 + 32, rb);
          stage(ra, c0);
          if (c0 + 32 < c_hi) {
            tmem_ld_wait();
            if (c0 + 64 < c_hi) tmem_ld_32x32(tcol + c0 + 64, ra);
            stage(rb, c0 + 32);
          }
        }
        tc_fence_before();
        __syncwarp();
        if (lane == 0) { mbar_arrive(tmem_empty + 8 * buf); tma_store_commit(); tma_store_wait_read(); }
        if (lt == 0 && threadIdx.x == 64) GTR(9);
        continue;
      }
#pragma unroll 1
      for (int c0 = c_lo; c0 < c_hi; c0 += 32) {
        uint32_t r[32];
        tmem_ld_32x32(tmem_base + ((uint32_t)(q * 32) << 16) + (uint32_t)(buf * BN + c0), r);
        const int nb = n0 + c0;
        const bool active = row_ok && nb < e.N;
        const bool fast = active && vec_ok && (nb + 32 <= e.N);
#pragma unroll
        for (int j = 0; j < 32; ++j) aux[j] = aux_next[j];
        if (aux_vec && c0 + 32 < c_hi && nb + 64 <= e.N) load32(aux_row + nb + 32, aux_next);
        tmem_ld_wait();
        if (c0 + 32 >= c_hi) {
          tc_fence_before();
          __syncwarp();
          if (lane == 0) mbar_arrive(tmem_empty + 8 * buf);
        }
        if (!active) continue;
        float v[32];
#pragma unroll
        for (int j = 0; j < 32; ++j) v[j] = __uint_as_float(r[j]);
        if (fast) {
          if (bias) {
#pragma unroll
            for (int j = 0; j < 32; j += 4) {
              const float4 b4 = *reinterpret_cast<const float4*>(sb + c0 + j);
              v[j] += b4.x; v[j + 1] += b4.y; v[j + 2] += b4.z; v[j + 3] += b4.w;
            }
          }
          if (e.relu) {
#pragma unroll
            for (int j = 0; j < 32; ++j) v[j] = fmaxf(v[j], 0.f);
          }
          if (mask_row) {
#pragma unroll
            for (int j = 0; j < 32; ++j) v[j] = aux[j] > 0.f ? v[j] * e.mask_scale : 0.f;
          }
          if (e.p_drop > 0.f) {
            const uint64_t idx0 = (uint64_t)m * e.N + nb;
            if (e.p_drop == 0.5f && (idx0 & 31) == 0) {
              const uint32_t kw = drop_word(e.drop_key ^ egot2_ep, idx0);
#pragma unroll
              for (int j = 0; j < 32; ++j) v[j] = (kw >> j) & 1u ? v[j] * inv_keep : 0.f;
            } else if (e.p_drop != 0.5f && (idx0 & 1) == 0) {
              float dm[32];
              drop_scale_n<32>(e.drop_key ^ egot2_ep, idx0, e.p_drop, inv_keep, dm);
#pragma unroll
              for (int j = 0; j < 32; ++j) v[j] *= dm[j];
            } else {
#pragma unroll
              for (int j = 0; j < 32; ++j) v[j] *= drop_scale(e.drop_key ^ egot2_ep, idx0 + j, e.p_drop, inv_keep);
            }
          }
          if (res_row) {
            if (mask_row) load32(res_row + nb, aux);
#pragma unroll
            for (int j = 0; j < 32; ++j) v[j] += aux[j];
          }
          if (e.accumulate) {
            if constexpr (sizeof(TO) == 4) {
              float* dst = (float*)crow_ptr + nb;
              if (e.atomic) {
#pragma unroll
                for (int j = 0; j < 32; j += 4) red_add_v4(dst + j, v[j], v[j + 1], v[j + 2], v[j + 3]);
              } else {
                float old[32];
                load32(dst, old);
#pragma unroll
                for (int j = 0; j < 32; ++j) v[j] += old[j];
                store32(dst, v);
              }
            }
          } else if (BN <= 128 && sizeof(TO) == 2 && (e.tma_store || e.ln_g)) {
            const int r = q * 32 + lane;
            const uint32_t srow = sOut + (uint32_t)(c0 >> 6) * 16384u + (uint32_t)r * 128u;
#pragma unroll
            for (int j = 0; j < 4; ++j) {
              uint32_t w[4];
#pragma unroll
              for (int k = 0; k < 4; ++k) {
                __nv_bfloat162 t = __floats2bfloat162_rn(v[8 * j + 2 * k], v[8 * j + 2 * k + 1]);
                w[k] = *reinterpret_cast<uint32_t*>(&t);
                if (e.ln_g) {
                  const float y0 = __uint_as_float(w[k] << 16), y1 = __uint_as_float(w[k] & 0xffff0000u);
                  ln_sum += y0 + y1;
                  ln_sq = fmaf(y0, y0, fmaf(y1, y1, ln_sq));
                }
              }
              sts128(srow + (uint32_t)(((((c0 & 63) >> 3) + j) ^ (r & 7)) << 4), w[0], w[1], w[2], w[3]);
            }
            if (!e.tma_store) store32(crow_ptr + nb, v);
          } else {
            store32(crow_ptr + nb, v);
          }
        } else {
#pragma unroll
          for (int j = 0; j < 32; ++j) {
            const int n = nb + j;
            if (n >= e.N) continue;
            float x = v[j];
            if (bias) x += sb[c0 + j];
            if (e.relu) x = fmaxf(x, 0.f);
            if (mask_row) x = to_f32(mask_row[n]) > 0.f ? x * e.mask_scale : 0.f;
            if (e.p_drop > 0.f) x *= drop_scale(e.drop_key ^ egot2_ep, (uint64_t)m * e.N + n, e.p_drop, inv_keep, e.drop_bit_mode != 0);
            if (res_row) x += to_f32(res_row[n]);
            if (e.accumulate) {
              if constexpr (sizeof(TO) == 4) {
                if (e.atomic) atomicAdd((float*)crow_ptr + n, x);
                else ((float*)crow_ptr)[n] += x;
              }
            } else {
              crow_ptr[n] = from_f32<TO>(x);
            }
          }
        }
      }
      if constexpr (BN == 128 && sizeof(TO) == 2) {
        if (e.ln_g && row_ok) {
          const float mean = ln_sum * (1.f / 128.f);
          const float rstd = rsqrtf(fmaxf(ln_sq * (1.f / 128.f) - mean * mean, 0.f) + e.ln_eps);
          const long long lrow = crow + e.ln_row0;
          if (e.ln_stat) { e.ln_stat[2 * lrow] = mean; e.ln_stat[2 * lrow + 1] = rstd; }
          bf16* orow = (bf16*)e.ln_out + crow * e.ldc;
          const float* trow = e.ln_table ? e.ln_table + (lrow % e.ln_table_rows) * 128 : nullptr;
          const float ln_keep = e.ln_p_drop > 0.f ? 1.f / (1.f - e.ln_p_drop) : 1.f;
          const int r = q * 32 + lane;
#pragma unroll 1
          for (int c0 = 0; c0 < 128; c0 += 32) {
            const uint32_t srow = sOut + (uint32_t)(c0 >> 6) * 16384u + (uint32_t)r * 128u;
#pragma unroll
            for (int j = 0; j < 4; ++j) {
              uint32_t w0, w1, w2, w3;
              asm volatile("ld.shared.v4.b32 {%0, %1, %2, %3}, [%4];" : "=r"(w0), "=r"(w1), "=r"(w2), "=r"(w3)
                           : "r"(srow + (uint32_t)(((((c0 & 63) >> 3) + j) ^ (r & 7)) << 4)));
              const uint32_t w[4] = {w0, w1, w2, w3};
              const int c = c0 + 8 * j;
              const float4 g0 = __ldg(reinterpret_cast<const float4*>(e.ln_g + c)), g1 = __ldg(reinterpret_cast<const float4*>(e.ln_g + c + 4));
              const float4 b0 = __ldg(reinterpret_cast<const float4*>(e.ln_b + c)), b1 = __ldg(reinterpret_cast<const float4*>(e.ln_b + c + 4));
              const float gg[8] = {g0.x, g0.y, g0.z, g0.w, g1.x, g1.y, g1.z, g1.w}, bb[8] = {b0.x, b0.y, b0.z, b0.w, b1.x, b1.y, b1.z, b1.w};
              float o[8];
#pragma unroll
              for (int k = 0; k < 4; ++k) {
                o[2 * k] = (__uint_as_float(w[k] << 16) - mean) * rstd * gg[2 * k] + bb[2 * k];
                o[2 * k + 1] = (__uint_as_float(w[k] & 0xffff0000u) - mean) * rstd * gg[2 * k + 1] + bb[2 * k + 1];
              }
              if (trow) {
                const float4 t0 = __ldg(reinterpret_cast<const float4*>(trow + c)), t1 = __ldg(reinterpret_cast<const float4*>(trow + c + 4));
                o[0] += t0.x; o[1] += t0.y; o[2] += t0.z; o[3] += t0.w; o[4] += t1.x; o[5] += t1.y; o[6] += t1.z; o[7] += t1.w;
              }
              if (e.ln_p_drop > 0.f) {
                { float dm[8]; drop_scale_n<8>(e.ln_drop_key ^ egot2_ep, (uint64_t)lrow * 128 + c, e.ln_p_drop, ln_keep, dm);
#pragma unroll
                  for (int k = 0; k < 8; ++k) o[k] *= dm[k]; }
              }
              uint4 pk;
              __nv_bfloat162 p0 = __floats2bfloat162_rn(o[0], o[1]), p1 = __floats2bfloat162_rn(o[2], o[3]);
              __nv_bfloat162 p2 = __floats2bfloat162_rn(o[4], o[5]), p3 = __floats2bfloat162_rn(o[6], o[7]);
              pk.x = *reinterpret_cast<uint32_t*>(&p0); pk.y = *reinterpret_cast<uint32_t*>(&p1);
              pk.z = *reinterpret_cast<uint32_t*>(&p2); pk.w = *reinterpret_cast<uint32_t*>(&p3);
              *reinterpret_cast<uint4*>(orow + c) = pk;
            }
          }
        }
      }
      if (lt == 0 && threadIdx.x == 64) GTR(9);
      if (BN <= 128 && e.tma_store) {
        fence_proxy_async();
        named_bar_sync(2, NTHREADS - 64);
        if (lt == 0 && threadIdx.x == 64) GTR(10);
        if (warp == 2 && lane == 0) {
#pragma unroll
          for (int h = 0; h < BN / 64; ++h) tma_store_2d(&tma_c, sOut + h * 16384, n0 + h * 64, m0);
          tma_store_commit();
        }
      }
    }
    if (e.tma_store && warp == 2 && lane == 0) tma_store_wait_all();
    if (threadIdx.x == 64) GTR(11);
  }
  tc_fence_before();
  __syncthreads();
  if (threadIdx.x == 0) GTR(12);
  if (warp == 1) {
    __syncwarp();
    if (one_tile) tmem_dealloc<BN>(tmem_base); else tmem_dealloc<2 * BN>(tmem_base);
    if (lane == 0) GTR(13);
  }
}

typedef CUresult (*EncodeTiledFn)(CUtensorMap*, CUtensorMapDataType, cuuint32_t, void*, const cuuint64_t*,
                                  const cuuint64_t*, const cuuint32_t*, const cuuint32_t*, CUtensorMapInterleave,
                                  CUtensorMapSwizzle, CUtensorMapL2promotion, CUtensorMapFloatOOBfill);

EncodeTiledFn encode_fn() {
  static EncodeTiledFn fn = nullptr;
  static bool tried = false;
  if (!tried) {
    tried = true;
    void* p = nullptr;
    cudaDriverEntryPointQueryResult qres;
    if (cudaGetDriverEntryPoint("cuTensorMapEncodeTiled", &p, cudaEnableDefault, &qres) == cudaSuccess &&
        qres == cudaDriverEntryPointSuccess)
      fn = (EncodeTiledFn)p;
  }
  return fn;
}

int make_map(CUtensorMap* map, const void* base, int inner, int rows, int ld, int box_inner, int box_rows) {
  EncodeTiledFn fn = encode_fn();
  EGOT2_CHECK(fn != nullptr, "cuTensorMapEncodeTiled not available from the driver");
  cuuint64_t dims[2] = {(cuuint64_t)inner, (cuuint64_t)rows};
  cuuint64_t strides[1] = {(cuuint64_t)ld * 2};
  cuuint32_t box[2] = {(cuuint32_t)box_inner, (cuuint32_t)box_rows};
  cuuint32_t estr[2] = {1, 1};
  CUresult r = fn(map, CU_TENSOR_MAP_DATA_TYPE_BFLOAT16, 2, const_cast<void*>(base), dims, strides, box, estr,
                  CU_TENSOR_MAP_INTERLEAVE_NONE, CU_TENSOR_MAP_SWIZZLE_128B, CU_TENSOR_MAP_L2_PROMOTION_L2_256B,
                  CU_TENSOR_MAP_FLOAT_OOB_FILL_NONE);
  EGOT2_CHECK(r == CUDA_SUCCESS, "cuTensorMapEncodeTiled failed (%d) inner=%d rows=%d ld=%d", (int)r, inner, rows, ld);
  return 0;
}

int make_map_f32(CUtensorMap* map, const void* base, int inner, int rows, int ld, int box_inner, int box_rows) {
  EncodeTiledFn fn = encode_fn();
  EGOT2_CHECK(fn != nullptr, "cuTensorMapEncodeTiled not available from the driver");
  cuuint64_t dims[2] = {(cuuint64_t)inner, (cuuint64_t)rows};
  cuuint64_t strides[1] = {(cuuint64_t)ld * 4};
  cuuint32_t box[2] = {(cuuint32_t)box_inner, (cuuint32_t)box_rows};
  cuuint32_t estr[2] = {1, 1};
  CUresult r = fn(map, CU_TENSOR_MAP_DATA_TYPE_FLOAT32, 2, const_cast<void*>(base), dims, strides, box, estr,
                  CU_TENSOR_MAP_INTERLEAVE_NONE, CU_TENSOR_MAP_SWIZZLE_128B, CU_TENSOR_MAP_L2_PROMOTION_L2_256B,
                  CU_TENSOR_MAP_FLOAT_OOB_FILL_NONE);
  EGOT2_CHECK(r == CUDA_SUCCESS, "cuTensorMapEncodeTiled(f32) failed (%d) inner=%d rows=%d ld=%d", (int)r, inner, rows, ld);
  return 0;
}

int make_map3(CUtensorMap* map, const void* base, int inner, int rpg, int groups, int ld, long long gstride_rows,
              int box_inner, int box_d, int box_g) {
  EncodeTiledFn fn = encode_fn();
  EGOT2_CHECK(fn != nullptr, "cuTensorMapEncodeTiled not available from the driver");
  cuuint64_t dims[3] = {(cuuint64_t)inner, (cuuint64_t)rpg, (cuuint64_t)groups};
  cuuint64_t strides[2] = {(cuuint64_t)ld * 2, (cuuint64_t)gstride_rows * ld * 2};
  cuuint32_t box[3] = {(cuuint32_t)box_inner, (cuuint32_t)box_d, (cuuint32_t)box_g};
  cuuint32_t estr[3] = {1, 1, 1};
  CUresult r = fn(map, CU_TENSOR_MAP_DATA_TYPE_BFLOAT16, 3, const_cast<void*>(base), dims, strides, box, estr,
                  CU_TENSOR_MAP_INTERLEAVE_NONE, CU_TENSOR_MAP_SWIZZLE_128B, CU_TENSOR_MAP_L2_PROMOTION_L2_256B,
                  CU_TENSOR_MAP_FLOAT_OOB_FILL_NONE);
  EGOT2_CHECK(r == CUDA_SUCCESS, "cuTensorMapEncodeTiled(3d) failed (%d) inner=%d rpg=%d groups=%d ld=%d", (int)r, inner,
              rpg, groups, ld);
  return 0;
}

struct KGroup { int on = 0, g = 1, dblocks = 1, kb_total = 0; };
#ifdef EGOT2_GEMM_TRACE
struct GTraceTag { char txt[96]; };
GTraceTag g_gtrace_tags[512];
int g_gtrace_n = 0;
#endif
static bool host_al16(const void* p) { return (reinterpret_cast<uintptr_t>(p) & 15) == 0; }

template <int BN, bool A_MN, bool B_MN, typename TO>
int launch(const GemmArgs& a, const CUtensorMap& ma, const CUtensorMap& mb, const KGroup& kg, cudaStream_t st) {
  constexpr int STAGES = TileCfg<BN, TO>::STAGES;
  constexpr size_t smem = 1024 + STAGES * (BM * BK * 2 + BN * BK * 2) + TileCfg<BN, TO>::OUT_BYTES + 16 * STAGES + 96 + 2 * BN * 4;
  static bool attr_set = false;
  auto kern = gemm_sm100_kernel<BN, A_MN, B_MN, TO>;
  if (!attr_set) {
    EGOT2_CUDA(cudaFuncSetAttribute(kern, cudaFuncAttributeMaxDynamicSharedMemorySize, (int)smem));
    attr_set = true;
  }
  EpiArgs e;
  e.M = a.M; e.N = a.N; e.C = a.C; e.ldc = a.ldc; e.c_rpg = a.c_rpg; e.c_gstride = a.c_gstride;
  e.bias = a.bias; e.relu = a.relu; e.mask = a.mask; e.ldm = a.ldm; e.mask_scale = a.mask_scale;
  e.p_drop = a.p_drop; e.drop_key = a.drop_key; e.drop_bit_mode = a.drop_bit_mode; e.residual = a.residual; e.ldr = a.ldr;
  e.accumulate = a.accumulate; e.atomic = a.split_k > 1;
  e.ln_g = a.ln_g; e.ln_b = a.ln_b; e.ln_eps = a.ln_eps; e.ln_out = a.ln_out; e.ln_stat = a.ln_stat; e.ln_table = a.ln_table;
  e.ln_table_rows = a.ln_table_rows > 0 ? a.ln_table_rows : 1; e.ln_row0 = a.ln_row0; e.ln_p_drop = a.ln_p_drop; e.ln_drop_key = a.ln_drop_key;
  e.k_grouped = kg.on; e.kg = kg.g; e.kdblocks = kg.dblocks;
  CUtensorMap mc = ma;
  e.tma_store = 0;
  if (BN <= 128 && sizeof(TO) == 2 && !a.accumulate && a.c_rpg == 0 && a.N % 32 == 0 && a.ldc % 8 == 0 && host_al16(a.C) &&
      (!a.mask || (host_al16(a.mask) && a.ldm % 8 == 0)) && (!a.residual || (host_al16(a.residual) && a.ldr % 8 == 0)) &&
      !(getenv("EGOT2_GEMM_TMASTORE") && getenv("EGOT2_GEMM_TMASTORE")[0] == '0')) {
    EGOT2_TRY(make_map(&mc, a.C, a.N, a.M, a.ldc, 64, 128));
    e.tma_store = 1;
  }
  const int kb_total = kg.on ? kg.kb_total : (a.K + BK - 1) / BK;
  int splits = a.split_k < 1 ? 1 : a.split_k;
  if (splits > kb_total) splits = kb_total;
  {
    const int nt = ((a.N + BN - 1) / BN) * ((a.M + BM - 1) / BM), slots = sm_count() * TileCfg<BN, TO>::MIN_CTAS;
    if (splits > 1 && nt * splits > slots) splits = slots / nt > 0 ? slots / nt : 1;
  }
  const int kb_per = (kb_total + splits - 1) / splits;
  splits = (kb_total + kb_per - 1) / kb_per;
  e.atomic = splits > 1 && a.split_stride == 0;
  e.split_stride = a.split_stride;
  static const bool tma_red_on = !(getenv("EGOT2_GEMM_TMARED") && getenv("EGOT2_GEMM_TMARED")[0] == '0');
  e.tma_red = 0;
  if (sizeof(TO) == 4 && tma_red_on && e.atomic && a.accumulate && !a.bias && !a.residual && !a.relu && !a.mask && a.p_drop <= 0.f &&
      a.c_rpg == 0 && a.N % 32 == 0 && a.ldc % 4 == 0 && host_al16(a.C) && (size_t)(BN / 32) * 16384 <= (size_t)STAGES * (BM * BK * 2 + BN * BK * 2)) {
    if (a.trans_c) EGOT2_TRY(make_map_f32(&mc, a.C, a.M, a.N, a.ldc, 32, 32));
    else EGOT2_TRY(make_map_f32(&mc, a.C, a.N, a.M, a.ldc, 32, 32));
    e.tma_red = 1;
  }
  e.trans_c = a.trans_c;
  if (a.trans_c && !e.tma_red) return -3;
  if (a.splits_out) *a.splits_out = splits;
  const int tiles_n = (a.N + BN - 1) / BN, num_tiles = tiles_n * ((a.M + BM - 1) / BM);
  int ctas = num_tiles;
  if (splits == 1) {
    const int slots = sm_count() * TileCfg<BN, TO>::MIN_CTAS;
    const int rounds = (num_tiles + slots - 1) / slots;
    ctas = (num_tiles + rounds - 1) / rounds;
  }
  dim3 grid(ctas, 1, splits);
  e.trace_slot = -1;
#ifdef EGOT2_GEMM_TRACE
  if (g_gtrace_n < 512) {
    snprintf(g_gtrace_tags[g_gtrace_n].txt, 96, "bn%d %s%s %s M%d N%d K%d grid(%d,%d) tma_store%d%s%s", BN, A_MN ? "mn" : "k", B_MN ? "mn" : "k",
             sizeof(TO) == 4 ? "f32" : "bf16", a.M, a.N, a.K, ctas, splits, e.tma_store, a.residual ? " +res" : "", a.p_drop > 0.f ? " +drop" : "");
    e.trace_slot = g_gtrace_n++;
  }
#endif
  ProfScope prof(st, "gemm_sm100<bn%d,%s%s,%s> M%d N%d K%d sk%d%s", BN, A_MN ? "mn" : "k", B_MN ? "mn" : "k",
                 sizeof(TO) == 4 ? "f32" : "bf16", a.M, a.N, a.K, splits, a.mask ? " +mask" : (a.residual ? " +res" : ""));
  ::egot2::launch(kern, grid, dim3(NTHREADS), smem, st, ma, mb, mc, e, kb_total, kb_per, tiles_n, num_tiles);
  EGOT2_LAUNCH_CHECK();
  return 0;
}

template <bool A_MN, bool B_MN, typename TO>
int pick_bn(const GemmArgs& a, int bn, const CUtensorMap& ma, const CUtensorMap& mb, const KGroup& kg, cudaStream_t st) {
  switch (bn) {
    case 64: return launch<64, A_MN, B_MN, TO>(a, ma, mb, kg, st);
    case 128: return launch<128, A_MN, B_MN, TO>(a, ma, mb, kg, st);
    default: return launch<256, A_MN, B_MN, TO>(a, ma, mb, kg, st);
  }
}

template <typename TO>
int pick_major(const GemmArgs& a, int bn, const CUtensorMap& ma, const CUtensorMap& mb, const KGroup& kg, cudaStream_t st) {
  if (!a.trans_a && a.trans_b) return pick_bn<false, false, TO>(a, bn, ma, mb, kg, st);
  if (!a.trans_a && !a.trans_b) return pick_bn<false, true, TO>(a, bn, ma, mb, kg, st);
  if (a.trans_a && !a.trans_b) return pick_bn<true, true, TO>(a, bn, ma, mb, kg, st);
  return pick_bn<true, false, TO>(a, bn, ma, mb, kg, st);
}

bool host_aligned16(const void* p) { return (reinterpret_cast<uintptr_t>(p) & 15) == 0; }

}

bool gemm_sm100_ln_ok(const GemmArgs& a) {
  if (!(getenv("EGOT2_GEMM_LN") && getenv("EGOT2_GEMM_LN")[0] == '1')) return false;
  return a.in_dtype == EGOT2_BF16 && a.out_dtype == EGOT2_BF16 && a.N == 128 && a.K >= 16 && !a.accumulate && a.split_k <= 1 &&
         a.split_stride == 0 && !a.mask && !a.trans_a && a.a_rpg == 0 && a.b_rpg == 0 && a.ldc == 128 && host_al16(a.C) &&
         host_al16(a.A) && host_al16(a.B) && a.lda % 8 == 0 && a.ldb % 8 == 0 && (!a.residual || (host_al16(a.residual) && a.ldr % 8 == 0)) &&
         (a.c_rpg == 0 || (a.c_rpg * 128 * 2) % 16 == 0);
}

#ifdef EGOT2_GEMM_TRACE
extern "C" int egot2_gemm_trace_dump() {
  static long long h[512][16];
  cudaDeviceSynchronize();
  cudaMemcpyFromSymbol(h, g_gtrace, sizeof(h));
  printf("# cycles since CTA entry: prologue | pdl_wait done | sync | tma first,last issued | mma saw first,last stage | epi saw acc | epi done | bar | stored | cta sync | dealloc\n");
  for (int i = 0; i < g_gtrace_n; ++i) {
    const long long t0 = h[i][0];
    printf("%-64s", g_gtrace_tags[i].txt);
    for (int k = 1; k < 14; ++k) printf(" %6lld", h[i][k] ? h[i][k] - t0 : -1LL);
    printf("\n");
  }
  g_gtrace_n = 0;
  fflush(stdout);
  return 0;
}
#endif

int gemm_sm100(const GemmArgs& a, cudaStream_t st) {
  if (a.in_dtype != EGOT2_BF16) return -1;
  if (a.ln_g && !gemm_sm100_ln_ok(a)) return -2;
  KGroup kg;
  if (a.a_rpg > 0 || a.b_rpg > 0) {
    if (!(a.trans_a && !a.trans_b)) return -1;
    const int rpg = a.a_rpg > 0 ? a.a_rpg : a.b_rpg;
    if ((a.a_rpg > 0 && a.b_rpg > 0 && a.a_rpg != a.b_rpg) || a.K % rpg) return -1;
    kg.on = 1;
    int dpad = 1;
    while (dpad < rpg && dpad < 64) dpad <<= 1;
    kg.g = 64 / dpad;
    kg.dblocks = (rpg + 63) / 64;
    const int groups = a.K / rpg;
    kg.kb_total = ((groups + kg.g - 1) / kg.g) * kg.dblocks;
  }
  if (a.M < 1 || a.N < 32 || a.K < 16) return -1;
  if (!host_aligned16(a.A) || !host_aligned16(a.B) || (a.lda % 8) || (a.ldb % 8)) return -1;
  if (a.accumulate && a.out_dtype != EGOT2_F32) return -1;
  if (a.trans_c && (!a.accumulate || a.out_dtype != EGOT2_F32 || a.split_k < 2 || a.split_stride > 0 || a.c_rpg > 0)) return -3;
  if (a.split_k > 1 && a.split_stride == 0 && (!a.accumulate || a.relu || a.mask || a.p_drop > 0.f)) return -1;
  if (a.split_stride > 0 && (a.accumulate || a.out_dtype != EGOT2_F32 || a.relu || a.mask || a.p_drop > 0.f || a.residual)) return -1;
  int bn = a.N <= 64 ? 64 : ((a.N <= 128 || a.K <= 512) ? 128 : ((a.N % 256 == 0 || a.N > 512) ? 256 : 128));
  {
    static const bool small_on = !(getenv("EGOT2_GEMM_BN_SMALL") && getenv("EGOT2_GEMM_BN_SMALL")[0] == '0');
    const long long mt = (a.M + BM - 1) / BM;
    if (small_on && !(a.accumulate && a.split_k > 1) && a.K >= 1024)
      while (bn > 64 && mt * ((a.N + bn - 1) / bn) < sm_count() / 4) bn >>= 1;
  }
  if (a.accumulate && a.split_k > 1) {
    const long long mt = (a.M + BM - 1) / BM;
    while (bn > 64 && mt * ((a.N + bn - 1) / bn) * a.split_k < sm_count()) bn >>= 1;
  }
  CUtensorMap ma, mb;
  if (kg.on) {
    const int rpg = a.a_rpg > 0 ? a.a_rpg : a.b_rpg, groups = a.K / rpg, dpad = 64 / kg.g;
    EGOT2_TRY(make_map3(&ma, a.A, a.M, rpg, groups, a.lda, a.a_rpg > 0 ? a.a_gstride : rpg, 64, dpad, kg.g));
    EGOT2_TRY(make_map3(&mb, a.B, a.N, rpg, groups, a.ldb, a.b_rpg > 0 ? a.b_gstride : rpg, 64, dpad, kg.g));
    if (a.out_dtype == EGOT2_F32) return pick_major<float>(a, bn, ma, mb, kg, st);
    return pick_major<bf16>(a, bn, ma, mb, kg, st);
  }
  if (!a.trans_a) EGOT2_TRY(make_map(&ma, a.A, a.K, a.M, a.lda, BK, BM));
  else EGOT2_TRY(make_map(&ma, a.A, a.M, a.K, a.lda, 64, BK));
  if (a.trans_b) EGOT2_TRY(make_map(&mb, a.B, a.K, a.N, a.ldb, BK, bn));
  else EGOT2_TRY(make_map(&mb, a.B, a.N, a.K, a.ldb, 64, BK));
  if (a.out_dtype == EGOT2_F32) return pick_major<float>(a, bn, ma, mb, kg, st);
  return pick_major<bf16>(a, bn, ma, mb, kg, st);
}

}
```

### egot2_b200/csrc/ops.h

```cpp
#pragma once
#include "common.cuh"

namespace egot2 {

struct GemmArgs {
  int M = 0, N = 0, K = 0;
  const void* A = nullptr; int lda = 0; int trans_a = 0;
  const void* B = nullptr; int ldb = 0; int trans_b = 0;
  void* C = nullptr;       int ldc = 0;
  int in_dtype = EGOT2_F32;
  int out_dtype = EGOT2_F32;
  int a_rpg = 0, a_gstride = 0;
  int b_rpg = 0, b_gstride = 0;
  int c_rpg = 0, c_gstride = 0;
  const float* bias = nullptr;
  int relu = 0;
  const void* mask = nullptr; int ldm = 0; float mask_scale = 1.f;
  float p_drop = 0.f; uint64_t drop_key = 0;
  int trans_c = 0;
  int drop_bit_mode = 0;
  const void* residual = nullptr; int ldr = 0;
  int accumulate = 0;
  int split_k = 1;
  long long split_stride = 0;
  int* splits_out = nullptr;
  const float* ln_g = nullptr; const float* ln_b = nullptr; float ln_eps = 1e-5f;
  void* ln_out = nullptr; float* ln_stat = nullptr; const float* ln_table = nullptr; int ln_table_rows = 0; int ln_row0 = 0;
  float ln_p_drop = 0.f; uint64_t ln_drop_key = 0;
};
bool gemm_sm100_ln_ok(const GemmArgs& a);
int gemm(const GemmArgs& a, cudaStream_t st);
int gemm_simt(const GemmArgs& a, cudaStream_t st);
int gemm_sm100(const GemmArgs& a, cudaStream_t st);
int suggest_split_k(int M, int N, int K);
const char* gemm_last_impl();

struct LayerNormArgs {
  int rows = 0, H = 0; int dtype = EGOT2_F32;
  const void* x = nullptr; const float* g = nullptr; const float* b = nullptr; float eps = 1e-5f;
  void* y = nullptr; float* stat = nullptr;
  const float* table = nullptr; int table_rows = 0;
  float p_drop = 0.f; uint64_t drop_key = 0;
  int x_is_f32 = 0;
};
int layernorm_fwd(const LayerNormArgs& a, cudaStream_t st);
struct LayerNormBwdArgs {
  int rows = 0, H = 0; int dtype = EGOT2_F32;
  const void* x = nullptr; const float* stat = nullptr; const float* g = nullptr;
  const void* dy = nullptr;
  void* dx = nullptr;
  const void* dres = nullptr;
  float* dg = nullptr; float* db = nullptr;
  int x_is_f32 = 0; int dx_is_f32 = 0; int dy_is_f32 = 0;
  float dy_p_drop = 0.f; uint64_t dy_drop_key = 0;
  float* dcol = nullptr;
  void* dx2 = nullptr; float dx2_p_drop = 0.f; uint64_t dx2_drop_key = 0;
};
int layernorm_bwd(const LayerNormBwdArgs& a, cudaStream_t st);

int attention_simt_fwd(int dtype, int B, int T, int H, int heads, const void* qkv, void* out, float* lse,
                       float p_drop, uint64_t drop_key, cudaStream_t st);
int attention_simt_bwd(int dtype, int B, int T, int H, int heads, const void* qkv, const void* out, const float* lse,
                       const void* dout, void* dqkv, float p_drop, uint64_t drop_key, void* ws, size_t ws_bytes,
                       cudaStream_t st);
bool attention_mma_supported(int dtype, int T, int H, int heads);
int attention_mma_fwd(int B, int T, int H, int heads, const void* qkv, void* out, float* lse, float p_drop,
                      uint64_t drop_key, cudaStream_t st);
int attention_mma_bwd(int B, int T, int H, int heads, const void* qkv, const void* out, const float* lse,
                      const void* dout, void* dqkv, float p_drop, uint64_t drop_key, cudaStream_t st);
bool attention_long_supported(int dtype, int T, int H, int heads);
int attention_long_fwd(int B, int T, int H, int heads, const void* qkv, void* out, float* lse, float p_drop, uint64_t drop_key,
                       cudaStream_t st);
int attention_long_bwd(int B, int T, int H, int heads, const void* qkv, const void* out, const float* lse, const void* dout,
                       void* dqkv, float p_drop, uint64_t drop_key, cudaStream_t st);
int attention_wide_fwd(int dtype, int B, int T, int H, int heads, const void* qkv, void* out, float* lse, float p_drop,
                       uint64_t drop_key, cudaStream_t st);
int attention_wide_bwd(int dtype, int B, int T, int H, int heads, const void* qkv, const void* out, const float* lse,
                       const void* dout, void* dqkv, float p_drop, uint64_t drop_key, cudaStream_t st);
int attention_fwd(int dtype, int B, int T, int H, int heads, const void* qkv, void* out, float* lse,
                  float p_drop, uint64_t drop_key, cudaStream_t st);
size_t attention_bwd_workspace(int dtype, int B, int T, int H, int heads);
int attention_bwd(int dtype, int B, int T, int H, int heads, const void* qkv, const void* out, const float* lse,
                  const void* dout, void* dqkv, float p_drop, uint64_t drop_key, void* ws, size_t ws_bytes,
                  cudaStream_t st);

struct SmallAttnArgs {
  int dtype = EGOT2_F32;
  int rows = 0, S = 0, M = 0, H = 0, heads = 0, causal = 0;
  const void* q = nullptr; int ldq = 0;
  const void* k = nullptr; const void* v = nullptr; int ldkv = 0;
  int kv_inner = 1, kv_outer = 0, kv_jstride = 1, kv_istride = 0;
  void* out = nullptr; int ldo = 0;
  float* lse = nullptr;
  float p_drop = 0.f; uint64_t drop_key = 0;
  const void* dout = nullptr;
  float* dq = nullptr; int ld_dq = 0;
  float* dk = nullptr; float* dv = nullptr; int ld_dkv = 0;
};
int small_attn_fwd(const SmallAttnArgs& a, cudaStream_t st);
int small_attn_bwd(const SmallAttnArgs& a, cudaStream_t st);

struct SegOut { int n = 0; int tokens[EGOT2_MAX_SEG] = {}; float* out[EGOT2_MAX_SEG] = {}; };
int table_grad(int dtype, int B, int T, int H, const void* dy, float* dtable, const SegOut& so, float p_drop, uint64_t drop_key,
               cudaStream_t st);
int colsum_accum(int dtype, int M, int N, const void* x, int ldx, int rpg, int gstride, float* out, cudaStream_t st);
int colsum_cast_bf16(int M, int N, const float* x, int ldx, void* y, int ldy, float* out, cudaStream_t st);
int dropout_inplace(int dtype, void* x, size_t n, float p, uint64_t key, cudaStream_t st);
int pool_fwd(int dtype, int B, int T, int H, int pool, int row_tokens, const void* x, float* pooled, cudaStream_t st);
int pool_bwd(int dtype, int B, int T, int H, int pool, int row_tokens, const float* dpooled, void* dx, cudaStream_t st);
int cast_f32_to(int dtype, const float* src, void* dst, size_t n, cudaStream_t st);
int cast_to_f32(int dtype, const void* src, float* dst, size_t n, cudaStream_t st);
int zero_f32(float* p, size_t n, cudaStream_t st);
int add_table(int dtype, size_t n, size_t table_elems, const void* z, const float* table, void* x, cudaStream_t st);
bool embed_finish_supported(int dtype, int H);
struct EmbedSrc {
  int n = 0; int tok_begin[EGOT2_MAX_SEG] = {}; int tokens[EGOT2_MAX_SEG] = {}; int splits[EGOT2_MAX_SEG] = {};
  const float* slab[EGOT2_MAX_SEG] = {}; const void* direct[EGOT2_MAX_SEG] = {};
  int direct_f32[EGOT2_MAX_SEG] = {};
};
int embed_finish(int B, int T, int H, const EmbedSrc& src, int drop_tokens, float p_feat, uint64_t key_feat, const float* g,
                 const float* b, float eps, const float* table, float p_embed, uint64_t key_embed, void* z, float* stat, void* x,
                 cudaStream_t st);
int sum_into_clear(float* dst, float* a, float* b, size_t n, cudaStream_t st);
int dropout_prefix_inplace(int dtype, void* x, size_t n, size_t period, size_t prefix, float p, uint64_t key, cudaStream_t st);
int cast_rows_f32_to_bf16(const float* src, int rows, int n, void* dst, int ld, cudaStream_t st);

bool ffn_fused_supported(int dtype, int H, int FF);
int ffn_fused_fwd(int M, int FF, const void* x1, const void* W1, const float* b1, const void* W2, const float* b2,
                  const float* ln_g, const float* ln_b, float eps, void* hid, void* hmask, void* y2, float* stat2, void* x_out,
                  float p_drop, uint64_t key_ffn, uint64_t key_drop2, float* scratch, cudaStream_t st);
size_t ffn_scratch_bytes(int M);
int ffn_fused_bwd_dx(int M, int FF, const void* d2, const void* d1, const void* hmask, const void* W1, const void* W2,
                     float p_drop, void* dhid, void* d3, float* scratch, float* db1, cudaStream_t st);

bool head_fused_supported(const egot2_head_desc& d);
int head_fused_fwd(const egot2_head_desc& d, const egot2_head_in& in, const egot2_head_out& out, cudaStream_t st);
int loss_reduce(const egot2_head_desc& d, int rows, const float* row_loss, float* loss, cudaStream_t st);
int head_fused_bwd(const egot2_head_desc& d, const egot2_head_in& in, const egot2_head_out& saved, float* dlogits, float dloss_scale,
                   void* dx, const egot2_head_grads& g, cudaStream_t st);

int pnr_metrics(int B, int n, const float* logits, const int64_t* label_idx, const float* label_onehot,
                const int64_t* sc_label, const double* fps, const int64_t* start, const int64_t* end, const int64_t* pnr,
                double* err_sec, long long* out_i64, double* out_f64, cudaStream_t st);
int loss_fwd(const egot2_head_desc& d, int rows, const float* logits, const int64_t* labels, const float* class_weight,
             float* row_loss, float* loss, int32_t* argmax, cudaStream_t st);
int loss_bwd(const egot2_head_desc& d, int rows, const float* logits, const int64_t* labels, const float* class_weight,
             const float* loss2, float dloss_scale, float* dlogits, cudaStream_t st);

__device__ __forceinline__ double block_sum_f64(double v, double* sh) {
#pragma unroll
  for (int o = 16; o > 0; o >>= 1) v += __shfl_down_sync(0xffffffffu, v, o);
  const int warp = threadIdx.x >> 5, nw = blockDim.x >> 5;
  __syncthreads();
  if ((threadIdx.x & 31) == 0) sh[warp] = v;
  __syncthreads();
  double s = 0.0;
  if (threadIdx.x == 0)
    for (int w = 0; w < nw; ++w) s += sh[w];
  return s;
}
__device__ __forceinline__ void grad_guard_finalize(double sumsq, float scale, egot2_grad_guard* guard, int32_t* step_dev) {
  const double tot = sqrt(sumsq) * fabs((double)scale);
  const float tn = (float)tot;
  guard->total_norm = tn;
  if (isfinite(tot)) {
    guard->coef = fminf(1.f, guard->max_norm / (tn + 1e-6f));
    guard->skip = 0;
  } else {
    guard->coef = 0.f;
    guard->skip = 1;
    guard->skipped += 1;
    if (step_dev) *step_dev -= 1;
  }
}

}
```

### include/egot2.h

```cpp
#ifndef EGOT2_H_
#define EGOT2_H_

#include <stddef.h>
#include <stdint.h>

#ifdef __cplusplus
extern "C" {
#endif

#define EGOT2_MAX_SEG 8
#define EGOT2_MAX_GROUPS 4

enum { EGOT2_F32 = 0, EGOT2_BF16 = 1 };
enum { EGOT2_LOSS_NONE = 0, EGOT2_LOSS_CE = 1, EGOT2_LOSS_BCE_SIGMOID = 2, EGOT2_LOSS_CE_GROUPS = 3 };

const char* egot2_version(void);
const char* egot2_last_error(void);
int egot2_sm_count(void);
uint64_t egot2_launch_count(void);
int egot2_dropout_epoch_enable(int on);
int egot2_dropout_epoch_set(uint64_t value, void* stream);
int egot2_dropout_epoch_advance(void* stream);
int egot2_dropout_epoch_host(uint64_t value);
int egot2_prof_enable(int on);
int egot2_side_defer(int on);
int egot2_side_join_all(void* stream);
int egot2_timeline_set(void* dev_buf);
int egot2_prof_report(char* buf_host, size_t buf_bytes);

typedef struct {
  int32_t dtype;
  int32_t feat_dtype;
  int32_t B, T, H;
  int32_t n_seg;
  int32_t seg_tokens[EGOT2_MAX_SEG];
  int32_t seg_in_dim[EGOT2_MAX_SEG];
  int32_t seg_offset[EGOT2_MAX_SEG];
  int32_t seg_has_proj[EGOT2_MAX_SEG];
  int32_t training;
  float p_feat;
  float p_embed;
  float ln_eps;
  uint64_t seed;
  int32_t no_ln;
  int32_t feat_drop_tokens;
} egot2_embed_desc;

typedef struct {
  const void* feat[EGOT2_MAX_SEG];
  const void* proj_w[EGOT2_MAX_SEG];
  const float* proj_b[EGOT2_MAX_SEG];
  const float* ln_g;
  const float* ln_b;
  const float* tok_table;
} egot2_embed_in;

typedef struct {
  void* z;
  float* stat;
  void* x;
} egot2_embed_out;

typedef struct {
  float* proj_w[EGOT2_MAX_SEG];
  float* proj_b[EGOT2_MAX_SEG];
  float* ln_g;
  float* ln_b;
  float* tok_table;
  float* dfeat[EGOT2_MAX_SEG];
  float* seg_embed[EGOT2_MAX_SEG];
} egot2_embed_grads;

size_t egot2_embed_workspace_bytes(const egot2_embed_desc* d, int backward);
int egot2_embed_fwd(const egot2_embed_desc* d, const egot2_embed_in* in, const egot2_embed_out* out,
                    void* workspace, size_t ws_bytes, void* stream);
int egot2_embed_bwd(const egot2_embed_desc* d, const egot2_embed_in* in, const egot2_embed_out* saved,
                    const void* dx , const egot2_embed_grads* g,
                    void* workspace, size_t ws_bytes, void* stream);

int egot2_hhi_tok_table_fwd(const float* task_embed , const float* pe, int32_t pe_len, int32_t n_seg,
                            const int32_t* seg_tokens_host, const int32_t* seg_task_id_host, int32_t H,
                            float* tok_table , void* stream);
int egot2_hhi_tok_table_bwd(const float* d_tok_table, int32_t n_seg, const int32_t* seg_tokens_host,
                            const int32_t* seg_task_id_host, int32_t H, float* d_task_embed , void* stream);

typedef struct {
  int32_t dtype;
  int32_t B, T, H, FF, heads;
  int32_t training;
  int32_t layer_index;
  float p_drop;
  float ln_eps;
  uint64_t seed;
} egot2_layer_desc;

typedef struct {
  const void* in_proj_w;
  const void* out_proj_w;
  const void* lin1_w;
  const void* lin2_w;
  const float *in_proj_b, *out_proj_b, *lin1_b, *lin2_b;
  const float *norm1_g, *norm1_b, *norm2_g, *norm2_b;
} egot2_layer_params;

typedef struct {
  float *in_proj_w, *out_proj_w, *lin1_w, *lin2_w;
  float *in_proj_b, *out_proj_b, *lin1_b, *lin2_b;
  float *norm1_g, *norm1_b, *norm2_g, *norm2_b;
} egot2_layer_grads;

typedef struct {
  void* qkv;
  void* attn;
  float* lse;
  void* y1;
  float* stat1;
  void* x1;
  void* hid;
  void* y2;
  float* stat2;
  void* hid_mask;
  float* ffn_scratch;
} egot2_layer_saved;

size_t egot2_ffn_scratch_bytes(int32_t M );
size_t egot2_encoder_layer_workspace_bytes(const egot2_layer_desc* d, int backward);
int egot2_encoder_layer_fwd(const egot2_layer_desc* d, const egot2_layer_params* p, const void* x_in,
                            void* x_out, const egot2_layer_saved* s, void* workspace, size_t ws_bytes,
                            void* stream);
int egot2_encoder_layer_bwd(const egot2_layer_desc* d, const egot2_layer_params* p, const void* x_in,
                            const egot2_layer_saved* s, void* dx_out, void* dx_in,
                            const egot2_layer_grads* g, void* workspace, size_t ws_bytes, void* stream);

typedef struct {
  int32_t dtype;
  int32_t B, T, D;
  int32_t heads, dim_head;
  int32_t mlp;
  int32_t layer_index;
  float ln_eps;
} egot2_vit_desc;

typedef struct {
  const void *qkv_w, *out_w;
  const void *ff1_w, *ff2_w;
  const float *norm_a_g, *norm_a_b;
  const float *norm_f_g, *norm_f_b;
  const float *ff1_b, *ff2_b;
} egot2_vit_params;

typedef struct {
  float *qkv_w, *out_w, *ff1_w, *ff2_w;
  float *norm_a_g, *norm_a_b, *norm_f_g, *norm_f_b, *ff1_b, *ff2_b;
} egot2_vit_grads;

typedef struct {
  void* h; float* stat_a;
  void* qkv;
  void* attn; float* lse;
  void* x1;
  void* h2; float* stat_f;
  void* u; void* act;
} egot2_vit_saved;

size_t egot2_vit_layer_workspace_bytes(const egot2_vit_desc* d);
int egot2_vit_layer_fwd(const egot2_vit_desc* d, const egot2_vit_params* p, const void* x_in , void* x_out,
                        const egot2_vit_saved* s, void* stream);
int egot2_vit_layer_bwd(const egot2_vit_desc* d, const egot2_vit_params* p, const void* x_in, const egot2_vit_saved* s,
                        const void* dx_out, void* dx_in, const egot2_vit_grads* g, void* workspace, size_t ws_bytes,
                        void* stream);

typedef struct {
  int32_t dtype;
  int32_t rows, S;
  int32_t mem_rows, M;
  int32_t kv_inner, kv_outer, kv_jstride, kv_istride;
  int32_t H, FF, heads;
  int32_t training, layer_index;
  float p_drop, ln_eps;
  uint64_t seed;
} egot2_decoder_desc;

typedef struct {
  const void *sa_in_w, *sa_out_w;
  const void *ca_in_w, *ca_out_w;
  const void *lin1_w, *lin2_w;
  const float *sa_in_b, *sa_out_b, *ca_in_b, *ca_out_b, *lin1_b, *lin2_b;
  const float *norm1_g, *norm1_b, *norm2_g, *norm2_b, *norm3_g, *norm3_b;
} egot2_decoder_params;

typedef struct {
  float *sa_in_w, *sa_out_w, *ca_in_w, *ca_out_w, *lin1_w, *lin2_w;
  float *sa_in_b, *sa_out_b, *ca_in_b, *ca_out_b, *lin1_b, *lin2_b;
  float *norm1_g, *norm1_b, *norm2_g, *norm2_b, *norm3_g, *norm3_b;
} egot2_decoder_grads;

typedef struct {
  void* qkv;
  void* a1;
  void* y1; float* stat1; void* x1;
  void* qc;
  void* kvc;
  void* a2;
  void* y2; float* stat2; void* x2;
  void* hid;
  void* y3; float* stat3;
} egot2_decoder_saved;

size_t egot2_decoder_layer_workspace_bytes(const egot2_decoder_desc* d);
int egot2_decoder_layer_fwd(const egot2_decoder_desc* d, const egot2_decoder_params* p, const void* y_in ,
                            const void* mem , void* y_out, const egot2_decoder_saved* s, void* stream);
int egot2_decoder_layer_bwd(const egot2_decoder_desc* d, const egot2_decoder_params* p, const void* y_in, const void* mem,
                            const egot2_decoder_saved* s, void* dy_out, void* dy_in, float* dmem,
                            const egot2_decoder_grads* g, void* workspace, size_t ws_bytes, void* stream);
int egot2_prompt_embed_fwd(int32_t dtype, int32_t rows, int32_t S, int32_t H, const int64_t* tokens,
                           const float* embedding, const float* pe, float p_drop, int32_t training, uint64_t seed,
                           void* y, void* stream);
int egot2_prompt_embed_bwd(int32_t dtype, int32_t rows, int32_t S, int32_t H, const int64_t* tokens, const void* dy,
                           float p_drop, int32_t training, uint64_t seed, float* d_embedding , void* stream);

typedef struct {
  int32_t dtype;
  int32_t B, T, H;
  int32_t pool;
  int32_t row_tokens;
  int32_t use_ln;
  int32_t n_out;
  int32_t loss;
  int32_t n_groups;
  int32_t group_size[EGOT2_MAX_GROUPS];
  int32_t sub_rows;
  int32_t training;
  float p_head;
  float ln_eps;
  uint64_t seed;
} egot2_head_desc;

typedef struct {
  const void* x;
  const float *ln_g, *ln_b;
  const void* w;
  const float* b;
  const int64_t* labels;
  const float* class_weight;
} egot2_head_in;

typedef struct {
  float* pooled;
  float* stat;
  void* g;
  float* logits;
  float* loss;
  int32_t* argmax;
  float* row_loss;
} egot2_head_out;

typedef struct {
  float *ln_g, *ln_b, *w, *b;
} egot2_head_grads;

int egot2_head_rows(const egot2_head_desc* d);
int egot2_head_loss_fwd(const egot2_head_desc* d, const egot2_head_in* in, const egot2_head_out* out, void* stream);
int egot2_head_loss_bwd(const egot2_head_desc* d, const egot2_head_in* in, const egot2_head_out* saved,
                        float* dlogits , float dloss_scale,
                        void* dx , const egot2_head_grads* g,
                        void* workspace, size_t ws_bytes, void* stream);
size_t egot2_head_workspace_bytes(const egot2_head_desc* d);

int egot2_slowfast_pool_fwd(const void* in, int32_t in_dtype, int32_t B, int32_t C, int32_t Tin, int32_t hw,
                            int32_t Tout, void* out, int32_t out_dtype, void* stream);
int egot2_cast_f32_to_bf16(const float* src, void* dst, size_t n, void* stream);
int egot2_sum_into_f32(float* dst, float* a, float* b, size_t n, void* stream);
int egot2_cast_bf16_to_f32(const void* src, float* dst, size_t n, void* stream);
int egot2_adam_step(float* param, const float* grad, float* exp_avg, float* exp_avg_sq, size_t n, float lr,
                    float beta1, float beta2, float eps, float weight_decay, int32_t step, float grad_scale,
                    void* stream);
int egot2_adam_step_fused(float* param, float* grad, float* exp_avg, float* exp_avg_sq, size_t n, float lr,
                          float beta1, float beta2, float eps, float weight_decay, int32_t step, float grad_scale,
                          void* shadow_bf16, int32_t zero_grad, void* stream);
int egot2_adam_step_fused_dev(float* param, float* grad, float* exp_avg, float* exp_avg_sq, size_t n, float lr,
                              float beta1, float beta2, float eps, float weight_decay, const int32_t* step_dev,
                              float grad_scale, void* shadow_bf16, int32_t zero_grad, void* stream);
int egot2_adamw_step_fused(float* param, float* grad, float* exp_avg, float* exp_avg_sq, size_t n, float lr,
                           float beta1, float beta2, float eps, float weight_decay, int32_t step, float grad_scale,
                           void* shadow_bf16, int32_t zero_grad, void* stream);

enum { EGOT2_LR_CONSTANT = 0, EGOT2_LR_COSINE = 1, EGOT2_LR_STEPS = 2 };
typedef struct {
  int32_t kind, n_milestones;
  int64_t warmup_steps, total_steps;
  double base_lr, warmup_start_lr, end_lr;
  int64_t milestones[8];
  double factors[9];
} egot2_lr_sched;
int egot2_opt_advance(int32_t* step_dev, const egot2_lr_sched* sched, float* lr_dev, void* stream);
int egot2_adam_step_fused_sched(float* param, float* grad, float* exp_avg, float* exp_avg_sq, size_t n, const float* lr_dev,
                                float beta1, float beta2, float eps, float weight_decay, const int32_t* step_dev,
                                float grad_scale, void* shadow_bf16, int32_t zero_grad, int32_t decoupled, void* stream);

typedef struct {
  float max_norm;
  float total_norm;
  float coef;
  int32_t skip;
  int32_t skipped;
} egot2_grad_guard;
size_t egot2_grad_norm_workspace_bytes(void);
int egot2_grad_norm(const float* grad, size_t n, float grad_scale, egot2_grad_guard* guard, int32_t* step_dev, void* workspace,
                    size_t ws_bytes, void* stream);
int egot2_adam_step_fused_guard(float* param, float* grad, float* exp_avg, float* exp_avg_sq, size_t n, float lr,
                                const float* lr_dev, float beta1, float beta2, float eps, float weight_decay,
                                const int32_t* step_dev, float grad_scale, void* shadow_bf16, int32_t zero_grad,
                                int32_t decoupled, const egot2_grad_guard* guard, void* stream);

typedef struct {
  int32_t world, rank;
  int64_t numel;
  void* slab[8];
  int64_t off_param, off_grad;
  int64_t off_shadow;
  int64_t off_flags;
  float* exp_avg; float* exp_avg_sq;
  float lr, beta1, beta2, eps, weight_decay;
  int32_t step;
  const int32_t* step_dev;
  int32_t decoupled;
  int32_t zero_grads_remote;
  const float* lr_dev;
  egot2_grad_guard* guard;
} egot2_dp_desc;
int egot2_peer_alloc(size_t bytes, void** ptr);
int egot2_peer_free(void* ptr);
int egot2_peer_handle_bytes(void);
int egot2_peer_export(void* ptr, void* handle_out);
int egot2_peer_import(const void* handle, void** ptr);
int egot2_peer_unimport(void* ptr);
size_t egot2_dp_flag_bytes(void);
int egot2_dp_reduce_adam(const egot2_dp_desc* d, void* stream);
int egot2_dp_reduce_adam_range(const egot2_dp_desc* d, int64_t lo, int64_t hi, int32_t channel, void* stream);

int egot2_pnr_metrics(int32_t B, int32_t n, const float* logits, const int64_t* label_idx, const float* label_onehot,
                      const int64_t* sc_label, const double* fps, const int64_t* start_frame, const int64_t* end_frame,
                      const int64_t* pnr_frame, double* err_sec, int64_t* out_counts, double* out_dist_sum, void* stream);

int egot2_segment_softmax_mean(int32_t n_seg, int32_t n_cls, const float* logits, const int32_t* seg_offsets, float* out,
                               void* stream);
int egot2_row_softmax(int64_t rows, int32_t n, const float* in, float* out, void* stream);
int egot2_topk_correct(int32_t N, int32_t C, const float* preds, const int64_t* labels, int32_t n_k, const int32_t* ks_host,
                       int64_t* correct, void* stream);
int egot2_edit_distance_prefix(int32_t N, int32_t Z, int32_t K, const int64_t* preds, const int64_t* labels, int32_t* min_dist,
                               int64_t* sum_min, void* stream);

int egot2_gemm(int32_t dtype, int32_t M, int32_t N, int32_t K, const void* A, int32_t trans_a, const void* B,
               int32_t trans_b, const float* bias, int32_t relu, void* C, int32_t c_is_f32, int32_t accumulate,
               void* stream);
const char* egot2_gemm_last_impl(void);
int egot2_layernorm_fwd(int32_t dtype, int32_t rows, int32_t H, const void* x, const float* g, const float* b,
                        float eps, void* y, float* stat, void* stream);
int egot2_attention_fwd(int32_t dtype, int32_t B, int32_t T, int32_t H, int32_t heads, const void* qkv, void* out,
                        float* lse, float p_drop, int32_t training, uint64_t seed, void* stream);
int egot2_attention_bwd(int32_t dtype, int32_t B, int32_t T, int32_t H, int32_t heads, const void* qkv,
                        const void* out, const float* lse, const void* dout, void* dqkv, float p_drop,
                        int32_t training, uint64_t seed, void* workspace, size_t ws_bytes, void* stream);

size_t egot2_attention_bwd_workspace_bytes(int32_t dtype, int32_t B, int32_t T, int32_t H, int32_t heads);
int egot2_pool_fwd(int32_t dtype, int32_t B, int32_t T, int32_t H, int32_t pool, int32_t row_tokens, const void* x,
                   float* pooled, void* stream);
int egot2_pool_bwd(int32_t dtype, int32_t B, int32_t T, int32_t H, int32_t pool, int32_t row_tokens,
                   const float* dpooled, void* dx, void* stream);

#ifdef __cplusplus
}
#endif
#endif
```

Before: 779,000.

## Fuse FFN lin1/lin2 weight-gradient GEMMs into one persistent paired launch

Adds a paired-GEMM path to the SM100 kernel: one persistent launch walks work units drawn from two GEMMs (FFN dW2 and dW1 weight gradients, one of them in swapped/transposed-C form), each with its own TMA maps. Split-K is planned per unit across the grid, and some pipeline stages are given over to a reduction buffer. The goal is to drop a separate launch and side-stream fork and to fill SMs better when each wgrad alone is too small. The cost is a more complex kernel with extra tensor-map parameters, fewer stages in the reduction case, and less overlap of dW2 with the dx computation, since dW2 now waits for dhid.

```diff
diff --git a/egot2_b200/_lib.py b/egot2_b200/_lib.py
--- a/egot2_b200/_lib.py
+++ b/egot2_b200/_lib.py
@@ -203,6 +203,7 @@
     "egot2_adam_step_fused_guard": (C.c_int, [vp, vp, vp, vp, sz, f32, vp, f32, f32, f32, f32, vp, f32, vp, i32, i32, vp, vp]),
     "egot2_gemm": (C.c_int, [i32, i32, i32, i32, vp, i32, vp, i32, vp, i32, vp, i32, i32, vp]),
     "egot2_gemm_last_impl": (C.c_char_p, []),
+    "egot2_wgrad_ffn": (C.c_int, [i32, i32, i32, i32, vp, vp, vp, vp, vp, vp, vp]),
     "egot2_layernorm_fwd": (C.c_int, [i32, i32, i32, vp, vp, vp, f32, vp, vp, vp]),
     "egot2_attention_fwd": (C.c_int, [i32, i32, i32, i32, i32, vp, vp, vp, f32, i32, u64, vp]),
     "egot2_attention_bwd": (C.c_int, [i32, i32, i32, i32, i32, vp, vp, vp, vp, vp, f32, i32, u64, vp, sz, vp]),
diff --git a/egot2_b200/csrc/api.cu b/egot2_b200/csrc/api.cu
--- a/egot2_b200/csrc/api.cu
+++ b/egot2_b200/csrc/api.cu
@@ -271,27 +271,51 @@
   return 0;
 }
 
-int wgrad(int dtype, int rows, int n_out, int k_in, const void* dY, int ld_dy, int dy_rpg, int dy_gs, const void* X,
-          int ld_x, int x_rpg, int x_gs, float* dW, cudaStream_t st, int share = 1) {
+bool wgrad_swap(int dtype, int n_out, int k_in, int dy_rpg, int x_rpg, int share) {
   static const bool swap_on = !env_is("EGOT2_WGRAD_SWAP", "0");
-  if (swap_on && dtype == EGOT2_BF16 && gemm_impl_mode() == 0 && k_in <= 128 && n_out >= 512 && !dy_rpg && !x_rpg && share == 1) {
-    GemmArgs t;
-    t.M = k_in; t.N = n_out; t.K = rows;
-    t.A = X; t.lda = ld_x; t.trans_a = 1;
-    t.B = dY; t.ldb = ld_dy; t.trans_b = 0;
-    t.C = dW; t.ldc = k_in; t.trans_c = 1; t.in_dtype = dtype; t.out_dtype = EGOT2_F32; t.accumulate = 1;
-    t.split_k = suggest_split_k(t.M, t.N, t.K);
-    const int rc = t.split_k >= 2 ? gemm_sm100(t, st) : -3;
-    if (rc >= 0) return rc;
-  }
+  return swap_on && dtype == EGOT2_BF16 && gemm_impl_mode() == 0 && k_in <= 128 && n_out >= 512 && !dy_rpg && !x_rpg && share == 1;
+}
+GemmArgs wgrad_args(bool swap, int dtype, int rows, int n_out, int k_in, const void* dY, int ld_dy, int dy_rpg, int dy_gs,
+                    const void* X, int ld_x, int x_rpg, int x_gs, float* dW, int share) {
   GemmArgs g;
-  g.M = n_out; g.N = k_in; g.K = rows;
-  g.A = dY; g.lda = ld_dy; g.trans_a = 1; g.a_rpg = dy_rpg; g.a_gstride = dy_gs;
-  g.B = X; g.ldb = ld_x; g.trans_b = 0; g.b_rpg = x_rpg; g.b_gstride = x_gs;
+  if (swap) {
+    g.M = k_in; g.N = n_out; g.K = rows;
+    g.A = X; g.lda = ld_x; g.trans_a = 1;
+    g.B = dY; g.ldb = ld_dy; g.trans_b = 0;
+    g.trans_c = 1;
+  } else {
+    g.M = n_out; g.N = k_in; g.K = rows;
+    g.A = dY; g.lda = ld_dy; g.trans_a = 1; g.a_rpg = dy_rpg; g.a_gstride = dy_gs;
+    g.B = X; g.ldb = ld_x; g.trans_b = 0; g.b_rpg = x_rpg; g.b_gstride = x_gs;
+  }
   g.C = dW; g.ldc = k_in; g.in_dtype = dtype; g.out_dtype = EGOT2_F32; g.accumulate = 1;
   g.split_k = suggest_split_k(g.M, g.N, g.K);
   if (share > 1) g.split_k = g.split_k / share > 0 ? g.split_k / share : 1;
-  return gemm(g, st);
+  return g;
+}
+int wgrad(int dtype, int rows, int n_out, int k_in, const void* dY, int ld_dy, int dy_rpg, int dy_gs, const void* X,
+          int ld_x, int x_rpg, int x_gs, float* dW, cudaStream_t st, int share = 1) {
+  if (wgrad_swap(dtype, n_out, k_in, dy_rpg, x_rpg, share)) {
+    const GemmArgs t = wgrad_args(true, dtype, rows, n_out, k_in, dY, ld_dy, dy_rpg, dy_gs, X, ld_x, x_rpg, x_gs, dW, share);
+    const int rc = t.split_k >= 2 ? gemm_sm100(t, st) : -3;
+    if (rc >= 0) return rc;
+  }
+  return gemm(wgrad_args(false, dtype, rows, n_out, k_in, dY, ld_dy, dy_rpg, dy_gs, X, ld_x, x_rpg, x_gs, dW, share), st);
+}
+
+bool wgrad_ffn_pair_on(int dtype, int H, int FF) {
+  return wgrad_swap(dtype, FF, H, 0, 0, 1) && !wgrad_swap(dtype, H, FF, 0, 0, 1) && !env_is("EGOT2_WGRAD_PERSIST", "0");
+}
+int wgrad_ffn(int dtype, int rows, int H, int FF, const void* d2, const void* hid, const void* dhid, const void* x1, float* dW2,
+              float* dW1, cudaStream_t st) {
+  if (wgrad_ffn_pair_on(dtype, H, FF)) {
+    const GemmArgs a = wgrad_args(wgrad_swap(dtype, H, FF, 0, 0, 1), dtype, rows, H, FF, d2, H, 0, 0, hid, FF, 0, 0, dW2, 1);
+    const GemmArgs b = wgrad_args(wgrad_swap(dtype, FF, H, 0, 0, 1), dtype, rows, FF, H, dhid, FF, 0, 0, x1, H, 0, 0, dW1, 1);
+    const int rc = gemm_sm100_pair(a, b, st);
+    if (rc >= 0) return rc;
+  }
+  EGOT2_TRY(wgrad(dtype, rows, H, FF, d2, H, 0, 0, hid, FF, 0, 0, dW2, st));
+  return wgrad(dtype, rows, FF, H, dhid, FF, 0, 0, x1, H, 0, 0, dW1, st);
 }
 
 }
@@ -832,11 +856,12 @@
     EGOT2_TRY(layernorm_bwd(l, st));
   }
   static const bool late_wgrad = env_is("EGOT2_LATE_WGRAD", "1");
+  const bool ffn_pair = wgrad_ffn_pair_on(dt, H, FF);
   auto fork_dw2 = [&]() -> int {
     cudaStream_t ss = side_fork(st, sd0, 0);
     return wgrad(dt, M, H, FF, d2, H, 0, 0, s->hid, FF, 0, 0, g->lin2_w, ss);
   };
-  if (!late_wgrad) EGOT2_TRY(fork_dw2());
+  if (!late_wgrad && !ffn_pair) EGOT2_TRY(fork_dw2());
   const bool fused_dx = s->hid_mask && ffn_fused_supported(dt, H, FF) && !env_is("EGOT2_FFN", "unfused");
   if (fused_dx) {
     EGOT2_TRY(ffn_fused_bwd_dx(M, FF, d2, pd > 0.f ? w.d1 : nullptr, s->hid_mask, p->lin1_w, p->lin2_w, pd, w.dhid, w.d3, s->ffn_scratch,
@@ -851,7 +876,8 @@
   }
   auto fork_dw1 = [&]() -> int {
     cudaStream_t ss = side_fork(st, sd1, 1);
-    EGOT2_TRY(wgrad(dt, M, FF, H, w.dhid, FF, 0, 0, s->x1, H, 0, 0, g->lin1_w, ss));
+    if (ffn_pair) EGOT2_TRY(wgrad_ffn(dt, M, H, FF, d2, s->hid, w.dhid, s->x1, g->lin2_w, g->lin1_w, ss));
+    else EGOT2_TRY(wgrad(dt, M, FF, H, w.dhid, FF, 0, 0, s->x1, H, 0, 0, g->lin1_w, ss));
     if (!fused_dx) {
       cudaStream_t s2 = side_fork(st, sd2, 1);
       EGOT2_TRY(colsum_accum(dt, M, FF, w.dhid, FF, 0, 0, g->lin1_b, s2));
@@ -867,7 +893,10 @@
     l.dcol = g->out_proj_b;
     EGOT2_TRY(layernorm_bwd(l, st));
   }
-  if (late_wgrad) { EGOT2_TRY(fork_dw2()); EGOT2_TRY(fork_dw1()); }
+  if (late_wgrad) {
+    if (!ffn_pair) EGOT2_TRY(fork_dw2());
+    EGOT2_TRY(fork_dw1());
+  }
   {
     cudaStream_t ss = side_fork(st, sd2, 2);
     EGOT2_TRY(wgrad(dt, M, H, H, dyo, H, 0, 0, s->attn, H, 0, 0, g->out_proj_w, ss));
@@ -1014,6 +1043,11 @@
   return gemm(g, (cudaStream_t)stream);
 }
 
+extern "C" int egot2_wgrad_ffn(int32_t dtype, int32_t rows, int32_t H, int32_t FF, const void* d2, const void* hid,
+                               const void* dhid, const void* x1, float* dW2, float* dW1, void* stream) {
+  return wgrad_ffn(dtype, rows, H, FF, d2, hid, dhid, x1, dW2, dW1, (cudaStream_t)stream);
+}
+
 extern "C" int egot2_sum_into_f32(float* dst, float* a, float* b, size_t n, void* stream) {
   return sum_into_clear(dst, a, b, n, (cudaStream_t)stream);
 }
diff --git a/egot2_b200/csrc/gemm_sm100.cu b/egot2_b200/csrc/gemm_sm100.cu
--- a/egot2_b200/csrc/gemm_sm100.cu
+++ b/egot2_b200/csrc/gemm_sm100.cu
@@ -8,6 +8,16 @@
 namespace egot2 {
 
 using namespace sm100;
+
+SplitPlan plan_split_units(int tiles, int kb_total, int split_k, int slots) {
+  SplitPlan p;
+  int splits = split_k < 1 ? 1 : split_k;
+  if (splits > kb_total) splits = kb_total > 0 ? kb_total : 1;
+  if (splits > 1 && (long long)tiles * splits > slots) splits = slots / tiles > 0 ? slots / tiles : 1;
+  p.kb_per = kb_total > 0 ? (kb_total + splits - 1) / splits : 1;
+  p.splits = kb_total > 0 ? (kb_total + p.kb_per - 1) / p.kb_per : 1;
+  return p;
+}
 
 namespace {
 
@@ -34,6 +44,7 @@
   void* ln_out; float* ln_stat; const float* ln_table; int ln_table_rows; int ln_row0;
   float ln_p_drop; uint64_t ln_drop_key;
   int trans_c;
+  int trans_c2;
   int tma_red;
   int trace_slot;
 };
@@ -95,25 +106,35 @@
   static constexpr uint32_t OUT_BYTES = (BN <= 128 && sizeof(TO) == 2) ? 128 * BN * 2 : 0;
   static constexpr int STAGES = BN == 128 ? (OUT_BYTES ? 2 : 3) : (BN == 64 ? (OUT_BYTES ? 3 : 4) : 4);
   static constexpr int MIN_CTAS = BN == 256 ? 1 : 2;
+  static constexpr uint32_t STAGE_BYTES = (BM + BN) * BK * 2;
+  static constexpr uint32_t RED_BYTES = sizeof(TO) == 4 ? 4 * EPG * 2 * 4096 : 0;
+  static constexpr int PSTAGES = RED_BYTES ? STAGES - 1 : STAGES;
+  static constexpr uint32_t RING_BYTES = STAGES * STAGE_BYTES > PSTAGES * STAGE_BYTES + RED_BYTES
+                                             ? STAGES * STAGE_BYTES : PSTAGES * STAGE_BYTES + RED_BYTES;
 };
 __device__ __forceinline__ void sts128(uint32_t dst, uint32_t a, uint32_t b, uint32_t c, uint32_t d) {
   asm volatile("st.shared.v4.b32 [%0], {%1, %2, %3, %4};" ::"r"(dst), "r"(a), "r"(b), "r"(c), "r"(d) : "memory");
 }
 
 __device__ __forceinline__ void named_bar_sync(int id, int n) { asm volatile("bar.sync %0, %1;" ::"r"(id), "r"(n) : "memory"); }
+__device__ __forceinline__ void bulk_wait_read_1() { asm volatile("cp.async.bulk.wait_group.read 1;" ::: "memory"); }
 
 template <int BN, bool A_MN, bool B_MN, typename TO>
 __global__ void __launch_bounds__(NTHREADS, TileCfg<BN, TO>::MIN_CTAS)
 gemm_sm100_kernel(const __grid_constant__ CUtensorMap tma_a, const __grid_constant__ CUtensorMap tma_b,
-                  const __grid_constant__ CUtensorMap tma_c, const EpiArgs e, const int k_blocks_total, const int k_blocks_per_split, const int tiles_n, const int num_tiles) {
+                  const __grid_constant__ CUtensorMap tma_c, const __grid_constant__ CUtensorMap tma_a2,
+                  const __grid_constant__ CUtensorMap tma_b2, const __grid_constant__ CUtensorMap tma_c2, const EpiArgs e,
+                  const int k_blocks_total, const int k_blocks_per_split, const int tiles_n, const int num_tiles, const int num_units,
+                  const int units_per_gemm, const int stages, const int red_own) {
   constexpr uint32_t A_BYTES = BM * BK * 2;
   constexpr uint32_t B_BYTES = BN * BK * 2;
   constexpr int STAGES = TileCfg<BN, TO>::STAGES;
   extern __shared__ uint8_t smem_raw[];
   const uint32_t smem_base = (smem_u32(smem_raw) + 1023u) & ~1023u;
   const uint32_t sA = smem_base;
-  const uint32_t sB = sA + STAGES * A_BYTES;
-  const uint32_t sOut = sB + STAGES * B_BYTES;
+  const uint32_t sB = sA + stages * A_BYTES;
+  const uint32_t sRed = sB + stages * B_BYTES;
+  const uint32_t sOut = sA + TileCfg<BN, TO>::RING_BYTES;
   const uint32_t bars = sOut + TileCfg<BN, TO>::OUT_BYTES;
   const uint32_t full0 = bars, empty0 = bars + 8 * STAGES, tmem_full = bars + 16 * STAGES, tmem_empty = tmem_full + 16;
   const uint32_t tmem_slot = tmem_empty + 16;
@@ -121,9 +142,10 @@
   uint32_t* tmem_slot_ptr = reinterpret_cast<uint32_t*>(smem_raw + (tmem_slot - smem_u32(smem_raw)));
 
   const int warp = threadIdx.x >> 5, lane = threadIdx.x & 31;
-  const int kb_begin = blockIdx.z * k_blocks_per_split;
-  const int kb_end = min(k_blocks_total, kb_begin + k_blocks_per_split);
-  const int nkb = kb_end - kb_begin;
+  auto unit_v = [&](int u) { return u >= units_per_gemm ? u - units_per_gemm : u; };
+  auto unit_split = [&](int u) { return (int)blockIdx.z + unit_v(u) / num_tiles; };
+  auto unit_kb0 = [&](int u) { return unit_split(u) * k_blocks_per_split; };
+  auto unit_nkb = [&](int u) { return min(k_blocks_total, unit_kb0(u) + k_blocks_per_split) - unit_kb0(u); };
 
   pdl_launch_dependents();
   if (threadIdx.x == 0) GTR(0);
@@ -131,7 +153,8 @@
     tma_prefetch_desc(&tma_a);
     tma_prefetch_desc(&tma_b);
     if (e.tma_store || e.tma_red) tma_prefetch_desc(&tma_c);
-    for (int s = 0; s < STAGES; ++s) { mbar_init(full0 + 8 * s, 1); mbar_init(empty0 + 8 * s, 1); }
+    if (units_per_gemm < num_units) { tma_prefetch_desc(&tma_a2); tma_prefetch_desc(&tma_b2); tma_prefetch_desc(&tma_c2); }
+    for (int s = 0; s < stages; ++s) { mbar_init(full0 + 8 * s, 1); mbar_init(empty0 + 8 * s, 1); }
     for (int s = 0; s < 2; ++s) { mbar_init(tmem_full + 8 * s, 1); mbar_init(tmem_empty + 8 * s, 4 * EPG); }
     fence_barrier_init();
   }
@@ -152,11 +175,15 @@
   if (warp == 0) {
     if (lane == 0) {
       int it = 0;
-      for (int tile = blockIdx.x; tile < num_tiles; tile += gridDim.x) {
+      for (int u = blockIdx.x; u < num_units; u += gridDim.x) {
+        const int tile = unit_v(u) % num_tiles;
         const int m0 = (tile / tiles_n) * BM, n0 = (tile % tiles_n) * BN;
+        const int kb_begin = unit_kb0(u), nkb = unit_nkb(u);
+        const CUtensorMap* map_a = u < units_per_gemm ? &tma_a : &tma_a2;
+        const CUtensorMap* map_b = u < units_per_gemm ? &tma_b : &tma_b2;
         for (int i = 0; i < nkb; ++i, ++it) {
-          const int s = it % STAGES;
-          const uint32_t ph = (it / STAGES) & 1;
+          const int s = it % stages;
+          const uint32_t ph = (it / stages) & 1;
           mbar_wait(empty0 + 8 * s, ph ^ 1);
           mbar_expect_tx(full0 + 8 * s, A_BYTES + B_BYTES);
           const int kb = kb_begin + i;
@@ -164,24 +191,24 @@
           if (A_MN && B_MN && e.k_grouped) {
             const int grp = (kb / e.kdblocks) * e.kg, d0 = (kb % e.kdblocks) * 64;
 #pragma unroll
-            for (int j = 0; j < BM / 64; ++j) tma_load_3d(sA + s * A_BYTES + j * 8192, &tma_a, full0 + 8 * s, m0 + 64 * j, d0, grp);
-#pragma unroll
-            for (int j = 0; j < BN / 64; ++j) tma_load_3d(sB + s * B_BYTES + j * 8192, &tma_b, full0 + 8 * s, n0 + 64 * j, d0, grp);
+            for (int j = 0; j < BM / 64; ++j) tma_load_3d(sA + s * A_BYTES + j * 8192, map_a, full0 + 8 * s, m0 + 64 * j, d0, grp);
+#pragma unroll
+            for (int j = 0; j < BN / 64; ++j) tma_load_3d(sB + s * B_BYTES + j * 8192, map_b, full0 + 8 * s, n0 + 64 * j, d0, grp);
             continue;
           }
           if (!A_MN) {
-            tma_load_2d(sA + s * A_BYTES, &tma_a, full0 + 8 * s, k, m0);
+            tma_load_2d(sA + s * A_BYTES, map_a, full0 + 8 * s, k, m0);
           } else {
 #pragma unroll
-            for (int j = 0; j < BM / 64; ++j) tma_load_2d(sA + s * A_BYTES + j * 8192, &tma_a, full0 + 8 * s, m0 + 64 * j, k);
+            for (int j = 0; j < BM / 64; ++j) tma_load_2d(sA + s * A_BYTES + j * 8192, map_a, full0 + 8 * s, m0 + 64 * j, k);
           }
           if (!B_MN) {
-            tma_load_2d(sB + s * B_BYTES, &tma_b, full0 + 8 * s, k, n0);
+            tma_load_2d(sB + s * B_BYTES, map_b, full0 + 8 * s, k, n0);
           } else {
 #pragma unroll
-            for (int j = 0; j < BN / 64; ++j) tma_load_2d(sB + s * B_BYTES + j * 8192, &tma_b, full0 + 8 * s, n0 + 64 * j, k);
-          }
-          if (tile == (int)blockIdx.x && (i == 0 || i == nkb - 1)) GTR(i == 0 ? 4 : 5);
+            for (int j = 0; j < BN / 64; ++j) tma_load_2d(sB + s * B_BYTES + j * 8192, map_b, full0 + 8 * s, n0 + 64 * j, k);
+          }
+          if (u == (int)blockIdx.x && (i == 0 || i == nkb - 1)) GTR(i == 0 ? 4 : 5);
         }
       }
     }
@@ -189,13 +216,14 @@
     if (lane == 0) {
       constexpr uint32_t idesc = make_idesc_bf16(BM, BN, A_MN, B_MN);
       int it = 0, lt = 0;
-      for (int tile = blockIdx.x; tile < num_tiles; tile += gridDim.x, ++lt) {
+      for (int u = blockIdx.x; u < num_units; u += gridDim.x, ++lt) {
         const int buf = lt & 1;
+        const int nkb = unit_nkb(u);
         mbar_wait(tmem_empty + 8 * buf, ((lt >> 1) & 1) ^ 1);
         tc_fence_after();
         for (int i = 0; i < nkb; ++i, ++it) {
-          const int s = it % STAGES;
-          const uint32_t ph = (it / STAGES) & 1;
+          const int s = it % stages;
+          const uint32_t ph = (it / stages) & 1;
           mbar_wait(full0 + 8 * s, ph);
           if (lt == 0 && (i == 0 || i == nkb - 1)) GTR(i == 0 ? 6 : 7);
           tc_fence_after();
@@ -216,12 +244,15 @@
     const int q = warp & 3;
     const int c_lo = ((warp - 2) >> 2) * (BN / EPG), c_hi = c_lo + BN / EPG;
     const float inv_keep = e.p_drop > 0.f ? 1.f / (1.f - e.p_drop) : 1.f;
-    const bool first_split = blockIdx.z == 0;
-    const float* bias = first_split ? e.bias : nullptr;
-    const bool tma_red = sizeof(TO) == 4 && e.tma_red && gridDim.z > 1 && nkb > 0;
+    int red_box = 0;
     int lt = 0;
-    for (int tile = blockIdx.x; tile < num_tiles; tile += gridDim.x, ++lt) {
+    for (int u = blockIdx.x; u < num_units; u += gridDim.x, ++lt) {
       const int buf = lt & 1;
+      const int tile = unit_v(u) % num_tiles, split = sizeof(TO) == 4 ? unit_split(u) : 0;
+      const int nkb = sizeof(TO) == 4 ? unit_nkb(u) : k_blocks_total;
+      const bool first_split = split == 0;
+      const float* bias = first_split ? e.bias : nullptr;
+      const bool tma_red = sizeof(TO) == 4 && e.tma_red && nkb > 0;
       const int m0 = (tile / tiles_n) * BM, n0 = (tile % tiles_n) * BN;
       const int m = m0 + q * 32 + lane;
       float* sb = sbias + buf * BN;
@@ -231,7 +262,7 @@
       }
       const bool row_ok = (m < e.M) && nkb > 0;
       const long long crow = row_ok ? remap(m, e.c_rpg, e.c_gstride) : 0;
-      TO* __restrict__ crow_ptr = (TO*)e.C + (long long)blockIdx.z * e.split_stride + crow * e.ldc;
+      TO* __restrict__ crow_ptr = (TO*)e.C + (long long)split * e.split_stride + crow * e.ldc;
       const TO* mask_row = e.mask ? (const TO*)e.mask + (long long)(row_ok ? m : 0) * e.ldm : nullptr;
       const TO* res_row = (e.residual && first_split) ? (const TO*)e.residual + (long long)(row_ok ? m : 0) * e.ldr : nullptr;
       const bool vec_ok = aligned16(crow_ptr) && aligned16(mask_row) && aligned16(res_row);
@@ -249,10 +280,17 @@
       float ln_sum = 0.f, ln_sq = 0.f;
       if (tma_red) {
         const int rr = q * 32 + lane;
+        const bool trans_c = u < units_per_gemm ? e.trans_c : e.trans_c2;
+        const CUtensorMap* map_c = u < units_per_gemm ? &tma_c : &tma_c2;
         uint32_t ra[32], rb[32];
         auto stage = [&](const uint32_t (&r)[32], int c0) {
-          const uint32_t wbox = sA + (uint32_t)(c0 >> 5) * 16384u + (uint32_t)(q * 32) * 128u;
-          if (e.trans_c) {
+          const uint32_t wbox = red_own ? sRed + (uint32_t)(warp - 2) * 8192u + (uint32_t)(red_box++ & 1) * 4096u
+                                        : sA + (uint32_t)(c0 >> 5) * 16384u + (uint32_t)(q * 32) * 128u;
+          if (red_own) {
+            if (lane == 0) bulk_wait_read_1();
+            __syncwarp();
+          }
+          if (trans_c) {
 #pragma unroll
             for (int j = 0; j < 32; ++j)
               asm volatile("st.shared.b32 [%0], %1;" ::"r"(wbox + (uint32_t)j * 128u + (uint32_t)((((lane >> 2) ^ (j & 7)) << 4) | ((lane & 3) << 2))), "r"(r[j]) : "memory");
@@ -264,9 +302,10 @@
           fence_proxy_async();
           __syncwarp();
           if (lane == 0 && n0 + c0 < e.N) {
-            if (e.trans_c) tma_reduce_add_2d(&tma_c, wbox, m0 + q * 32, n0 + c0);
-            else tma_reduce_add_2d(&tma_c, wbox, n0 + c0, m0 + q * 32);
-          }
+            if (trans_c) tma_reduce_add_2d(map_c, wbox, m0 + q * 32, n0 + c0);
+            else tma_reduce_add_2d(map_c, wbox, n0 + c0, m0 + q * 32);
+          }
+          if (red_own && lane == 0) tma_store_commit();
         };
         const uint32_t tcol = tmem_base + ((uint32_t)(q * 32) << 16) + (uint32_t)(buf * BN);
         tmem_ld_32x32(tcol + c_lo, ra);
@@ -283,7 +322,10 @@
         }
         tc_fence_before();
         __syncwarp();
-        if (lane == 0) { mbar_arrive(tmem_empty + 8 * buf); tma_store_commit(); tma_store_wait_read(); }
+        if (lane == 0) {
+          mbar_arrive(tmem_empty + 8 * buf);
+          if (!red_own) { tma_store_commit(); tma_store_wait_read(); }
+        }
         if (lt == 0 && threadIdx.x == 64) GTR(9);
         continue;
       }
@@ -463,6 +505,7 @@
       }
     }
     if (e.tma_store && warp == 2 && lane == 0) tma_store_wait_all();
+    if (red_own && lane == 0) tma_store_wait_read();
     if (threadIdx.x == 64) GTR(11);
   }
   tc_fence_before();
@@ -545,10 +588,11 @@
 #endif
 static bool host_al16(const void* p) { return (reinterpret_cast<uintptr_t>(p) & 15) == 0; }
 
+struct Pair { const GemmArgs* a; const CUtensorMap* ma; const CUtensorMap* mb; };
 template <int BN, bool A_MN, bool B_MN, typename TO>
-int launch(const GemmArgs& a, const CUtensorMap& ma, const CUtensorMap& mb, const KGroup& kg, cudaStream_t st) {
+int launch(const GemmArgs& a, const CUtensorMap& ma, const CUtensorMap& mb, const KGroup& kg, cudaStream_t st, const Pair* pair) {
   constexpr int STAGES = TileCfg<BN, TO>::STAGES;
-  constexpr size_t smem = 1024 + STAGES * (BM * BK * 2 + BN * BK * 2) + TileCfg<BN, TO>::OUT_BYTES + 16 * STAGES + 96 + 2 * BN * 4;
+  constexpr size_t smem = 1024 + TileCfg<BN, TO>::RING_BYTES + TileCfg<BN, TO>::OUT_BYTES + 16 * STAGES + 96 + 2 * BN * 4;
   static bool attr_set = false;
   auto kern = gemm_sm100_kernel<BN, A_MN, B_MN, TO>;
   if (!attr_set) {
@@ -572,65 +616,81 @@
     e.tma_store = 1;
   }
   const int kb_total = kg.on ? kg.kb_total : (a.K + BK - 1) / BK;
-  int splits = a.split_k < 1 ? 1 : a.split_k;
-  if (splits > kb_total) splits = kb_total;
-  {
-    const int nt = ((a.N + BN - 1) / BN) * ((a.M + BM - 1) / BM), slots = sm_count() * TileCfg<BN, TO>::MIN_CTAS;
-    if (splits > 1 && nt * splits > slots) splits = slots / nt > 0 ? slots / nt : 1;
-  }
-  const int kb_per = (kb_total + splits - 1) / splits;
-  splits = (kb_total + kb_per - 1) / kb_per;
+  const int tiles_n = (a.N + BN - 1) / BN, num_tiles = tiles_n * ((a.M + BM - 1) / BM);
+  const int slots = sm_count() * TileCfg<BN, TO>::MIN_CTAS;
+  const SplitPlan plan = plan_split_units(num_tiles, kb_total, a.split_k, slots);
+  const int splits = plan.splits;
   e.atomic = splits > 1 && a.split_stride == 0;
   e.split_stride = a.split_stride;
   static const bool tma_red_on = !(getenv("EGOT2_GEMM_TMARED") && getenv("EGOT2_GEMM_TMARED")[0] == '0');
+  auto red_ok = [&](const GemmArgs& g) {
+    return sizeof(TO) == 4 && tma_red_on && e.atomic && g.accumulate && !g.bias && !g.residual && !g.relu && !g.mask &&
+           g.p_drop <= 0.f && g.c_rpg == 0 && g.N % 32 == 0 && g.ldc % 4 == 0 && host_al16(g.C) &&
+           (size_t)(BN / 32) * 16384 <= (size_t)STAGES * (BM * BK * 2 + BN * BK * 2);
+  };
+  auto red_map = [&](const GemmArgs& g, CUtensorMap* m) {
+    return g.trans_c ? make_map_f32(m, g.C, g.M, g.N, g.ldc, 32, 32) : make_map_f32(m, g.C, g.N, g.M, g.ldc, 32, 32);
+  };
   e.tma_red = 0;
-  if (sizeof(TO) == 4 && tma_red_on && e.atomic && a.accumulate && !a.bias && !a.residual && !a.relu && !a.mask && a.p_drop <= 0.f &&
-      a.c_rpg == 0 && a.N % 32 == 0 && a.ldc % 4 == 0 && host_al16(a.C) && (size_t)(BN / 32) * 16384 <= (size_t)STAGES * (BM * BK * 2 + BN * BK * 2)) {
-    if (a.trans_c) EGOT2_TRY(make_map_f32(&mc, a.C, a.M, a.N, a.ldc, 32, 32));
-    else EGOT2_TRY(make_map_f32(&mc, a.C, a.N, a.M, a.ldc, 32, 32));
+  if (red_ok(a)) {
+    EGOT2_TRY(red_map(a, &mc));
     e.tma_red = 1;
   }
   e.trans_c = a.trans_c;
   if (a.trans_c && !e.tma_red) return -3;
+  CUtensorMap mc2 = mc;
+  e.trans_c2 = 0;
+  if (pair) {
+    if (!e.tma_red || !red_ok(*pair->a)) return -1;
+    EGOT2_TRY(red_map(*pair->a, &mc2));
+    e.trans_c2 = pair->a->trans_c;
+  }
   if (a.splits_out) *a.splits_out = splits;
-  const int tiles_n = (a.N + BN - 1) / BN, num_tiles = tiles_n * ((a.M + BM - 1) / BM);
   int ctas = num_tiles;
   if (splits == 1) {
-    const int slots = sm_count() * TileCfg<BN, TO>::MIN_CTAS;
     const int rounds = (num_tiles + slots - 1) / slots;
     ctas = (num_tiles + rounds - 1) / rounds;
   }
-  dim3 grid(ctas, 1, splits);
+  const int units_per_gemm = pair ? num_tiles * splits : num_tiles;
+  const int num_units = pair ? 2 * units_per_gemm : num_tiles;
+  if (pair) ctas = units_per_gemm;
+  const int red_own = pair ? 1 : 0;
+  const int stages = pair ? TileCfg<BN, TO>::PSTAGES : STAGES;
+  dim3 grid(ctas, 1, pair ? 1 : splits);
   e.trace_slot = -1;
 #ifdef EGOT2_GEMM_TRACE
   if (g_gtrace_n < 512) {
-    snprintf(g_gtrace_tags[g_gtrace_n].txt, 96, "bn%d %s%s %s M%d N%d K%d grid(%d,%d) tma_store%d%s%s", BN, A_MN ? "mn" : "k", B_MN ? "mn" : "k",
-             sizeof(TO) == 4 ? "f32" : "bf16", a.M, a.N, a.K, ctas, splits, e.tma_store, a.residual ? " +res" : "", a.p_drop > 0.f ? " +drop" : "");
+    snprintf(g_gtrace_tags[g_gtrace_n].txt, 96, "bn%d %s%s %s M%d N%d K%d grid(%d,%d) units%d tma_store%d%s%s", BN, A_MN ? "mn" : "k", B_MN ? "mn" : "k",
+             sizeof(TO) == 4 ? "f32" : "bf16", a.M, a.N, a.K, ctas, (int)grid.z, num_units * (int)grid.z, e.tma_store, a.residual ? " +res" : "", a.p_drop > 0.f ? " +drop" : "");
     e.trace_slot = g_gtrace_n++;
   }
 #endif
-  ProfScope prof(st, "gemm_sm100<bn%d,%s%s,%s> M%d N%d K%d sk%d%s", BN, A_MN ? "mn" : "k", B_MN ? "mn" : "k",
-                 sizeof(TO) == 4 ? "f32" : "bf16", a.M, a.N, a.K, splits, a.mask ? " +mask" : (a.residual ? " +res" : ""));
-  ::egot2::launch(kern, grid, dim3(NTHREADS), smem, st, ma, mb, mc, e, kb_total, kb_per, tiles_n, num_tiles);
+  ProfScope prof(st, "gemm_sm100<bn%d,%s%s,%s> M%d N%d K%d sk%d%s%s", BN, A_MN ? "mn" : "k", B_MN ? "mn" : "k",
+                 sizeof(TO) == 4 ? "f32" : "bf16", a.M, a.N, a.K, splits, pair ? " x2" : "",
+                 a.mask ? " +mask" : (a.residual ? " +res" : ""));
+  ::egot2::launch(kern, grid, dim3(NTHREADS), smem, st, ma, mb, mc, pair ? *pair->ma : ma, pair ? *pair->mb : mb, mc2, e, kb_total,
+                  plan.kb_per, tiles_n, num_tiles, num_units, units_per_gemm, stages, red_own);
   EGOT2_LAUNCH_CHECK();
   return 0;
 }
 
 template <bool A_MN, bool B_MN, typename TO>
-int pick_bn(const GemmArgs& a, int bn, const CUtensorMap& ma, const CUtensorMap& mb, const KGroup& kg, cudaStream_t st) {
+int pick_bn(const GemmArgs& a, int bn, const CUtensorMap& ma, const CUtensorMap& mb, const KGroup& kg, cudaStream_t st,
+            const Pair* pair) {
   switch (bn) {
-    case 64: return launch<64, A_MN, B_MN, TO>(a, ma, mb, kg, st);
-    case 128: return launch<128, A_MN, B_MN, TO>(a, ma, mb, kg, st);
-    default: return launch<256, A_MN, B_MN, TO>(a, ma, mb, kg, st);
+    case 64: return launch<64, A_MN, B_MN, TO>(a, ma, mb, kg, st, pair);
+    case 128: return launch<128, A_MN, B_MN, TO>(a, ma, mb, kg, st, pair);
+    default: return launch<256, A_MN, B_MN, TO>(a, ma, mb, kg, st, pair);
   }
 }
 
 template <typename TO>
-int pick_major(const GemmArgs& a, int bn, const CUtensorMap& ma, const CUtensorMap& mb, const KGroup& kg, cudaStream_t st) {
-  if (!a.trans_a && a.trans_b) return pick_bn<false, false, TO>(a, bn, ma, mb, kg, st);
-  if (!a.trans_a && !a.trans_b) return pick_bn<false, true, TO>(a, bn, ma, mb, kg, st);
-  if (a.trans_a && !a.trans_b) return pick_bn<true, true, TO>(a, bn, ma, mb, kg, st);
-  return pick_bn<true, false, TO>(a, bn, ma, mb, kg, st);
+int pick_major(const GemmArgs& a, int bn, const CUtensorMap& ma, const CUtensorMap& mb, const KGroup& kg, cudaStream_t st,
+               const Pair* pair = nullptr) {
+  if (!a.trans_a && a.trans_b) return pick_bn<false, false, TO>(a, bn, ma, mb, kg, st, pair);
+  if (!a.trans_a && !a.trans_b) return pick_bn<false, true, TO>(a, bn, ma, mb, kg, st, pair);
+  if (a.trans_a && !a.trans_b) return pick_bn<true, true, TO>(a, bn, ma, mb, kg, st, pair);
+  return pick_bn<true, false, TO>(a, bn, ma, mb, kg, st, pair);
 }
 
 bool host_aligned16(const void* p) { return (reinterpret_cast<uintptr_t>(p) & 15) == 0; }
@@ -663,14 +723,13 @@
 }
 #endif
 
-int gemm_sm100(const GemmArgs& a, cudaStream_t st) {
-  if (a.in_dtype != EGOT2_BF16) return -1;
-  if (a.ln_g && !gemm_sm100_ln_ok(a)) return -2;
+namespace {
+bool kgroup_of(const GemmArgs& a, KGroup* out) {
   KGroup kg;
   if (a.a_rpg > 0 || a.b_rpg > 0) {
-    if (!(a.trans_a && !a.trans_b)) return -1;
+    if (!(a.trans_a && !a.trans_b)) return false;
     const int rpg = a.a_rpg > 0 ? a.a_rpg : a.b_rpg;
-    if ((a.a_rpg > 0 && a.b_rpg > 0 && a.a_rpg != a.b_rpg) || a.K % rpg) return -1;
+    if ((a.a_rpg > 0 && a.b_rpg > 0 && a.a_rpg != a.b_rpg) || a.K % rpg) return false;
     kg.on = 1;
     int dpad = 1;
     while (dpad < rpg && dpad < 64) dpad <<= 1;
@@ -679,23 +738,46 @@
     const int groups = a.K / rpg;
     kg.kb_total = ((groups + kg.g - 1) / kg.g) * kg.dblocks;
   }
+  *out = kg;
+  return true;
+}
+
+int operand_maps(const GemmArgs& a, int bn, CUtensorMap* ma, CUtensorMap* mb) {
+  if (!a.trans_a) EGOT2_TRY(make_map(ma, a.A, a.K, a.M, a.lda, BK, BM));
+  else EGOT2_TRY(make_map(ma, a.A, a.M, a.K, a.lda, 64, BK));
+  if (a.trans_b) EGOT2_TRY(make_map(mb, a.B, a.K, a.N, a.ldb, BK, bn));
+  else EGOT2_TRY(make_map(mb, a.B, a.N, a.K, a.ldb, 64, BK));
+  return 0;
+}
+
+int choose_bn(const GemmArgs& a) {
+  int bn = a.N <= 64 ? 64 : ((a.N <= 128 || a.K <= 512) ? 128 : ((a.N % 256 == 0 || a.N > 512) ? 256 : 128));
+  {
+    static const bool small_on = !(getenv("EGOT2_GEMM_BN_SMALL") && getenv("EGOT2_GEMM_BN_SMALL")[0] == '0');
+    const long long mt = (a.M + BM - 1) / BM;
+    if (small_on && !(a.accumulate && a.split_k > 1) && a.K >= 1024)
+      while (bn > 64 && mt * ((a.N + bn - 1) / bn) < sm_count() / 4) bn >>= 1;
+  }
+  if (a.accumulate && a.split_k > 1) {
+    const long long mt = (a.M + BM - 1) / BM;
+    while (bn > 64 && mt * ((a.N + bn - 1) / bn) * a.split_k < sm_count()) bn >>= 1;
+  }
+  return bn;
+}
+}
+
+int gemm_sm100(const GemmArgs& a, cudaStream_t st) {
+  if (a.in_dtype != EGOT2_BF16) return -1;
+  if (a.ln_g && !gemm_sm100_ln_ok(a)) return -2;
+  KGroup kg;
+  if (!kgroup_of(a, &kg)) return -1;
   if (a.M < 1 || a.N < 32 || a.K < 16) return -1;
   if (!host_aligned16(a.A) || !host_aligned16(a.B) || (a.lda % 8) || (a.ldb % 8)) return -1;
   if (a.accumulate && a.out_dtype != EGOT2_F32) return -1;
   if (a.trans_c && (!a.accumulate || a.out_dtype != EGOT2_F32 || a.split_k < 2 || a.split_stride > 0 || a.c_rpg > 0)) return -3;
   if (a.split_k > 1 && a.split_stride == 0 && (!a.accumulate || a.relu || a.mask || a.p_drop > 0.f)) return -1;
   if (a.split_stride > 0 && (a.accumulate || a.out_dtype != EGOT2_F32 || a.relu || a.mask || a.p_drop > 0.f || a.residual)) return -1;
-  int bn = a.N <= 64 ? 64 : ((a.N <= 128 || a.K <= 512) ? 128 : ((a.N % 256 == 0 || a.N > 512) ? 256 : 128));
-  {
-    static const bool small_on = !(getenv("EGOT2_GEMM_BN_SMALL") && getenv("EGOT2_GEMM_BN_SMALL")[0] == '0');
-    const long long mt = (a.M + BM - 1) / BM;
-    if (small_on && !(a.accumulate && a.split_k > 1) && a.K >= 1024)
-      while (bn > 64 && mt * ((a.N + bn - 1) / bn) < sm_count() / 4) bn >>= 1;
-  }
-  if (a.accumulate && a.split_k > 1) {
-    const long long mt = (a.M + BM - 1) / BM;
-    while (bn > 64 && mt * ((a.N + bn - 1) / bn) * a.split_k < sm_count()) bn >>= 1;
-  }
+  const int bn = choose_bn(a);
   CUtensorMap ma, mb;
   if (kg.on) {
     const int rpg = a.a_rpg > 0 ? a.a_rpg : a.b_rpg, groups = a.K / rpg, dpad = 64 / kg.g;
@@ -704,12 +786,27 @@
     if (a.out_dtype == EGOT2_F32) return pick_major<float>(a, bn, ma, mb, kg, st);
     return pick_major<bf16>(a, bn, ma, mb, kg, st);
   }
-  if (!a.trans_a) EGOT2_TRY(make_map(&ma, a.A, a.K, a.M, a.lda, BK, BM));
-  else EGOT2_TRY(make_map(&ma, a.A, a.M, a.K, a.lda, 64, BK));
-  if (a.trans_b) EGOT2_TRY(make_map(&mb, a.B, a.K, a.N, a.ldb, BK, bn));
-  else EGOT2_TRY(make_map(&mb, a.B, a.N, a.K, a.ldb, 64, BK));
+  EGOT2_TRY(operand_maps(a, bn, &ma, &mb));
   if (a.out_dtype == EGOT2_F32) return pick_major<float>(a, bn, ma, mb, kg, st);
   return pick_major<bf16>(a, bn, ma, mb, kg, st);
 }
 
-}
+int gemm_sm100_pair(const GemmArgs& a, const GemmArgs& b, cudaStream_t st) {
+  for (const GemmArgs* g : {&a, &b}) {
+    if (g->in_dtype != EGOT2_BF16 || g->out_dtype != EGOT2_F32 || !g->accumulate || g->split_k < 2 || g->split_stride > 0 ||
+        g->a_rpg > 0 || g->b_rpg > 0 || g->ln_g || !host_aligned16(g->A) || !host_aligned16(g->B) || (g->lda % 8) || (g->ldb % 8))
+      return -1;
+  }
+  if (a.M != b.M || a.N != b.N || a.K != b.K || a.trans_a != b.trans_a || a.trans_b != b.trans_b || a.split_k != b.split_k ||
+      a.M < 1 || a.N < 32 || a.K < 16)
+    return -1;
+  const int bn = choose_bn(a);
+  CUtensorMap ma, mb, ma2, mb2;
+  EGOT2_TRY(operand_maps(a, bn, &ma, &mb));
+  EGOT2_TRY(operand_maps(b, bn, &ma2, &mb2));
+  const KGroup kg;
+  const Pair pair{&b, &ma2, &mb2};
+  return pick_major<float>(a, bn, ma, mb, kg, st, &pair);
+}
+
+}
diff --git a/egot2_b200/csrc/ops.h b/egot2_b200/csrc/ops.h
--- a/egot2_b200/csrc/ops.h
+++ b/egot2_b200/csrc/ops.h
@@ -33,6 +33,9 @@
 int gemm_simt(const GemmArgs& a, cudaStream_t st);
 int gemm_sm100(const GemmArgs& a, cudaStream_t st);
 int suggest_split_k(int M, int N, int K);
+struct SplitPlan { int splits = 1, kb_per = 1; };
+SplitPlan plan_split_units(int tiles, int kb_total, int split_k, int slots);
+int gemm_sm100_pair(const GemmArgs& a, const GemmArgs& b, cudaStream_t st);
 const char* gemm_last_impl();
 
 struct LayerNormArgs {
diff --git a/include/egot2.h b/include/egot2.h
--- a/include/egot2.h
+++ b/include/egot2.h
@@ -355,6 +355,8 @@
                int32_t trans_b, const float* bias, int32_t relu, void* C, int32_t c_is_f32, int32_t accumulate,
                void* stream);
 const char* egot2_gemm_last_impl(void);
+int egot2_wgrad_ffn(int32_t dtype, int32_t rows, int32_t H, int32_t FF, const void* d2, const void* hid, const void* dhid,
+                    const void* x1, float* dW2, float* dW1, void* stream);
 int egot2_layernorm_fwd(int32_t dtype, int32_t rows, int32_t H, const void* x, const float* g, const float* b,
                         float eps, void* y, float* stat, void* stream);
 int egot2_attention_fwd(int32_t dtype, int32_t B, int32_t T, int32_t H, int32_t heads, const void* qkv, void* out,
```

Result: slower. 769,000 (median of 6 runs) (-1.3%).
